# ActiveVisionLab/gaussctrl

Hardware: AMD Instinct MI355X
Metric: edited views/sec @512x512 (ControlNet denoise + splat render+bwd) (higher is better)
Workload: dtype bf16

## Files before the change

### gaussctrl_amd/csrc/dn_gemm.hip

```cpp
#include "dn_gemm_kernels.h"

namespace {

struct GemmVariant {
    int force_mt;
    int use8;
    int convsplit;
    bool no_wg2, no_persist, full_epilogue, no_lean_ln, tap_outer;
    int forced_pw, slice_mt, epi_abl;
    int undefined;
};
GemmVariant decode_variant(int kv)
{
    const auto bit = [kv](int b) { return (kv & b) != 0; };
    const auto field = [kv](int mask, int shift) { return (kv & mask) >> shift; };
    constexpr int flags = GC_GEMM_VAR_K4_ONLY | GC_GEMM_VAR_FORCE_K8 | GC_GEMM_VAR_NO_CONV_SLICES | GC_GEMM_VAR_NO_SMALL_CONV_SLICES | GC_GEMM_VAR_NO_WG2 |
                          GC_GEMM_VAR_NO_PERSIST | GC_GEMM_VAR_FULL_EPILOGUE | GC_GEMM_VAR_NO_LEAN_LN | GC_GEMM_VAR_TAP_OUTER;
    return {field(GC_GEMM_VAR_MT_MASK, GC_GEMM_VAR_MT_SHIFT), bit(GC_GEMM_VAR_K4_ONLY) ? 0 : bit(GC_GEMM_VAR_FORCE_K8) ? 2 : 1,
            bit(GC_GEMM_VAR_NO_CONV_SLICES) ? 0 : bit(GC_GEMM_VAR_NO_SMALL_CONV_SLICES) ? 1 : 2,
            bit(GC_GEMM_VAR_NO_WG2), bit(GC_GEMM_VAR_NO_PERSIST), bit(GC_GEMM_VAR_FULL_EPILOGUE), bit(GC_GEMM_VAR_NO_LEAN_LN), bit(GC_GEMM_VAR_TAP_OUTER),
            field(GC_GEMM_VAR_PW_MASK, GC_GEMM_VAR_PW_SHIFT), field(GC_GEMM_VAR_SLICE_MT_MASK, GC_GEMM_VAR_SLICE_MT_SHIFT), field(GC_GEMM_VAR_EPI_ABL_MASK, GC_GEMM_VAR_EPI_ABL_SHIFT),
            kv & ~(flags | GC_GEMM_VAR_MT_MASK | GC_GEMM_VAR_PW_MASK | GC_GEMM_VAR_SLICE_MT_MASK | GC_GEMM_VAR_EPI_ABL_MASK)};
}

int choose_splits(int64_t blocks, int nk)
{
    if (blocks >= 128 || nk < 32) return 1;
    int s = (int)((448 + blocks - 1) / blocks);
    if (s > nk / 8) s = nk / 8;
    if (s > 16) s = 16;
    return s < 2 ? 1 : s;
}

int choose_mt(int64_t M, int64_t N, int ntw, bool forced)
{
    const int64_t nbn = (N + 32 * ntw - 1) / (32 * ntw);
    if (((M + 127) / 128) * nbn < 96 && !forced) return 0;
    int best = 2;
    int64_t best_cost = -1;
    for (int mt = 2; mt <= 4; ++mt) {
        const int64_t tiles = ((M + 64 * mt - 1) / (64 * mt)) * nbn;
        const int64_t cost = ((tiles + 255) / 256) * (mt + 1);
        if (best_cost < 0 || cost < best_cost || (cost == best_cost && mt == 4)) { best = mt; best_cost = cost; }
    }
    return best;
}

int choose_pw(int64_t nbm, int64_t nbn, int64_t total_wgs, int conc, int64_t bm, int64_t bn, bool conv)
{
    int64_t r = total_wgs / 8 < 1 ? 1 : total_wgs / 8;
    if (r > conc) r = conc;
    const int64_t tiles = nbm * nbn;
    if (r >= tiles) return 0;
    const int64_t ca = conv ? bm : 9 * bm, cw = 9 * bn;
    int best = 0;
    int64_t best_cost = -1;
    for (int64_t pw = nbn; pw >= 1; --pw) {
        const int64_t per = nbm * pw;
        const int64_t cols = std::min<int64_t>(nbn, pw * ((r + per - 1) / per)), rows = std::min<int64_t>(nbm, (r + pw - 1) / pw);
        const int64_t cost = rows * ca + cols * cw;
        if (best_cost < 0 || cost < best_cost) { best = pw == nbn ? 0 : (int)pw; best_cost = cost; }
    }
    return best;
}

int pw_of(const gc_gemm_desc *d, const GemmVariant &v, int64_t nbm, int64_t nbn, int64_t total_wgs, int conc, int64_t bm, int64_t bn)
{
    if (v.forced_pw) return v.forced_pw - 1;
    return choose_pw(nbm, nbn, total_wgs, conc, bm, bn, d->mode == 1);
}

void plan(const gc_gemm_desc *d, int *ntw, int *splits, int *tps)
{
    *ntw = (d->N % 160 == 0 && d->N % 128 != 0 && !d->geglu) ? 5 : 4;
    if (d->softmax_keys > 0) *ntw = 5;
    const int bn = 32 * *ntw;
    const int64_t Msel = d->plan_rows > 0 ? d->plan_rows : d->M;
    const int64_t blocks = ((Msel + BM - 1) / BM) * ((d->N + bn - 1) / bn);
    const int nk = (int)((d->K + BK - 1) / BK);
    *splits = (d->geglu || d->w_set_rows > 0 || d->softmax_keys > 0) ? 1 : choose_splits(blocks, nk);
    *tps = (nk + *splits - 1) / *splits;
    *splits = (nk + *tps - 1) / *tps;
}


struct SelQ { int ntw, mt, splits, tps; };
void select_fp8(const gc_gemm_desc *d, const GemmVariant &v, SelQ *o, bool assume_ws)
{
    const int force_mt = v.force_mt;
    o->ntw = (d->N % 160 == 0 && d->N % 128 != 0 && !d->geglu) ? 5 : 4;
    int mt = force_mt ? force_mt : choose_mt(d->M, d->N, o->ntw, true);
    if (o->ntw == 5) mt = 2; else if (mt > 3) mt = 3;
    if (mt < 2) mt = 2;
    const int nkq = (int)(d->K / 128);
    o->splits = 1; o->tps = nkq;
    const bool plain = !d->geglu && !d->out_t && !d->out_fp8 && !d->out_f32 && d->out && !d->ln_row_stats && !d->out_row_stats && !d->out_group_stats && d->act == 0;
    const int64_t Msel = d->plan_rows > 0 ? d->plan_rows : d->M;
    const int64_t nbn = (d->N + 32 * o->ntw - 1) / (32 * o->ntw), tiles = ((Msel + 127) / 128) * nbn;
    if (plain && !force_mt && v.convsplit && tiles <= 128 && nkq >= 16) {
        int s = (int)std::min<int64_t>(tiles < 96 ? (256 + tiles - 1) / tiles : 256 / tiles, nkq / 8);
        if (s > 16) s = 16;
        if (s >= 2 && (assume_ws || (d->workspace && d->workspace_bytes >= sizeof(float) * (size_t)s * (size_t)d->M * (size_t)d->N))) {
            mt = 2; o->tps = (nkq + s - 1) / s; o->splits = (nkq + o->tps - 1) / o->tps;
        }
    }
    o->mt = mt;
}
}

extern "C" size_t gc_dn_gemm_workspace_bytes(const gc_gemm_desc *d)
{
    if (!d || d->M <= 0 || d->N <= 0 || d->K <= 0) return 0;
    if (d->fp8) {
        if (d->K % 128 != 0) return 0;
        const GemmVariant v = decode_variant(d->kernel_variant);
        SelQ q;
        select_fp8(d, v, &q, true);
        return q.splits > 1 ? sizeof(float) * (size_t)q.splits * (size_t)d->M * (size_t)d->N : 0;
    }
    int ntw, splits, tps;
    plan(d, &ntw, &splits, &tps);
    return splits > 1 ? sizeof(float) * (size_t)splits * (size_t)d->M * (size_t)d->N : 0;
}

namespace {
int ln_lean_kind(const gc_gemm_desc *d, const GemmVariant &v)
{
    if (v.no_lean_ln || d->fp8 || d->mode != 0 || d->K % 64 != 0 || d->out_group_stats || d->out_chan_parts || d->N < 4) return 0;
    if (d->out_row_stats && !d->ln_row_stats)
        return (!d->geglu && d->act == 0 && !d->out_f32 && !d->out_t && d->out && (!d->rowvec || d->rows_per_batch >= 256)) ? 1 : 0;
    if (d->ln_row_stats && !d->out_row_stats) return d->softmax_keys > 0 ? 3 : 2;
    return 0;
}
struct Sel { int mode, ntw, splits, tps, mt8; };
int select(const gc_gemm_desc *d, const GemmVariant &v, Sel *o, bool want_parts)
{
    int mode = 0;
    if (d->mode == 1) mode = (d->Cin % 64 == 0) ? 2 : 1;
    int ntw, splits, tps;
    plan(d, &ntw, &splits, &tps);
    if (splits > 1 && (!d->workspace || d->workspace_bytes < sizeof(float) * (size_t)splits * (size_t)d->M * (size_t)d->N)) {
        splits = 1; tps = (int)((d->K + BK - 1) / BK);
    }
    const int bn = 32 * ntw;
    const int64_t nbn = (d->N + bn - 1) / bn;
    const int nk_host = (int)((d->K + BK - 1) / BK);
    const int force_mt = v.force_mt, use8 = v.use8;
    o->mode = mode; o->ntw = ntw; o->splits = splits; o->tps = tps; o->mt8 = 0;
    if (use8 && d->zeros) {
        const int64_t Msel = d->plan_rows > 0 ? d->plan_rows : d->M;
        int mt = force_mt ? force_mt : choose_mt(Msel, d->N, ntw, use8 == 2);
        if (mt && !force_mt && Msel != d->M) mt = choose_mt(d->M, d->N, ntw, true);
        const int64_t tiles8 = ((Msel + 127) / 128) * nbn;
        const bool small = tiles8 < 96;
        if (!mt && mode == 0 && !force_mt) mt = 2;
        if (mode == 0 && !force_mt && ntw == 4 && d->K % 64 == 0 && !d->geglu && !d->out_t && !v.no_wg2 &&
            (!(d->ln_row_stats || d->out_row_stats || d->out_group_stats) || ln_lean_kind(d, v)) && !want_parts) {
            const int64_t t1 = ((d->M + 63) / 64) * nbn, t2 = ((d->M + 127) / 128) * nbn;
            if (mt == 2 && t2 <= 256 && t1 <= 512 && t1 > 128 && nk_host <= 24) mt = 1;
        }
        if (d->w_set_rows > 0 && mt) {
            int pick = 0;
            const int cand[5] = {mt, 4, 3, 2, (ntw == 4 && d->softmax_keys == 0) ? 1 : 2};
            for (int c = 0; c < 5 && !pick; ++c) if (d->w_set_rows % (64 * cand[c]) == 0) pick = cand[c];
            mt = pick ? pick : mt;
        }
        const bool want_split = !force_mt && use8 != 2 && !d->geglu && d->w_set_rows == 0 && d->softmax_keys == 0 && d->workspace && tiles8 <= 128 && (mode == 0 ? (!small || nk_host >= 24) : (v.convsplit >= (small ? 2 : 1)));
        int s8 = 1, tps8 = nk_host;
        if (want_split) {
            const bool img8 = mode != 0 && !small && d->Ho * d->Wo <= 64 && Msel % 256 == 0;
            const int mts = (v.slice_mt >= 2 && v.slice_mt <= 4) ? v.slice_mt : (img8 ? 4 : ((mode != 0 && !small) ? 3 : 2));
            const int64_t tiles_s = ((Msel + 64 * mts - 1) / (64 * mts)) * nbn;
            s8 = (int)std::min<int64_t>(std::max<int64_t>(256 / tiles_s, 2), nk_host / 12);
            if (s8 >= 2 && d->workspace_bytes >= sizeof(float) * (size_t)s8 * (size_t)d->M * (size_t)d->N) {
                mt = mts; tps8 = (nk_host + s8 - 1) / s8; s8 = (nk_host + tps8 - 1) / tps8;
            } else s8 = 1;
        }
        if (splits > 1 && s8 == 1 && !force_mt && use8 != 2) mt = 0;
        if (mt) { o->mt8 = mt; o->splits = s8; o->tps = tps8; }
    }
    return 0;
}
}

extern "C" int gc_dn_gemm_row_stat_slots(const gc_gemm_desc *d)
{
    if (!d || d->M <= 0 || d->N <= 0 || d->K <= 0) return 0;
    if (d->fp8) { const int ntw = (d->N % 160 == 0 && d->N % 128 != 0) ? 5 : 4; return (int)((d->N + 16 * ntw - 1) / (16 * ntw)); }
    const GemmVariant v = decode_variant(d->kernel_variant);
    Sel sel;
    select(d, v, &sel, false);
    return sel.splits > 1 ? (int)((d->N / 4 + 63) / 64) : (int)((d->N + 16 * sel.ntw - 1) / (16 * sel.ntw));
}

namespace {
void chan_parts_layout(const gc_gemm_desc *d, const GemmVariant &v, const Sel &sel, int64_t *rows, int *nslab, int *col_tile)
{
    *rows = 0; *nslab = 0; *col_tile = 0;
    const int64_t rpb = d->rows_per_batch;
    if (d->fp8) {
        SelQ q;
        select_fp8(d, v, &q, false);
        if (d->K % 128 != 0 || rpb < 256 || rpb % 32 != 0 || d->M % rpb != 0 || d->gn_groups < 1 || d->N % d->gn_groups != 0) return;
        const int64_t cpg = d->N / d->gn_groups;
        if (q.splits > 1) {
            if (cpg > 64) return;
            *rows = CS_RB; *nslab = (int)(rpb / CS_RB); *col_tile = 64;
            return;
        }
        const bool lean = d->mode == 1 && !d->upsample && !d->geglu && !d->out_t && !d->out_fp8 && !d->out_f32 && d->out && d->act == 0 &&
                          !d->ln_row_stats && !d->out_row_stats && !d->out_group_stats;
        const int64_t bm = 64 * q.mt;
        if (!lean || bm > rpb || cpg > 32 * q.ntw) return;
        *rows = bm;
        *nslab = (int)(rpb % bm == 0 ? rpb / bm : (rpb + bm - 1) / bm + 1);
        *col_tile = 32 * q.ntw;
        return;
    }
    if (d->geglu || d->act != 0 || d->out_t || !d->out || d->out_f32 || d->ln_row_stats || d->out_row_stats || d->out_group_stats) return;
    if (rpb < 256 || rpb % 32 != 0 || d->M % rpb != 0) return;
    if (d->gn_groups < 1 || d->N % d->gn_groups != 0) return;
    const int64_t cpg = d->N / d->gn_groups;
    if (sel.splits > 1) {
        if (cpg > 64) return;
        *rows = CS_RB; *nslab = (int)(rpb / CS_RB); *col_tile = 64;
        return;
    }
    if (!sel.mt8) return;
    if ((d->mode == 1 && d->upsample) || (d->mode == 0 && d->K % 64 != 0)) return;
    const int64_t bm = 64 * (sel.mt8 < 2 ? 2 : sel.mt8);
    if (bm > rpb || cpg > 32 * sel.ntw) return;
    *rows = bm;
    *nslab = (int)(rpb % bm == 0 ? rpb / bm : (rpb + bm - 1) / bm + 1);
    *col_tile = 32 * sel.ntw;
}
}

extern "C" int gc_dn_gemm_chan_parts_layout(const gc_gemm_desc *d, int64_t *rows_per_slab, int *nslab, int *col_tile)
{
    GC_REQUIRE(d && rows_per_slab && nslab && col_tile, "null argument");
    *rows_per_slab = 0; *nslab = 0; *col_tile = 0;
    if (d->M <= 0 || d->N <= 0 || d->K <= 0 || d->rows_per_batch <= 0) return GC_OK;
    const GemmVariant v = decode_variant(d->kernel_variant);
    Sel sel;
    select(d, v, &sel, true);
    chan_parts_layout(d, v, sel, rows_per_slab, nslab, col_tile);
    return GC_OK;
}

namespace {
struct Route { Sel sel; int lnk, persist; };
void route(const gc_gemm_desc *d, const GemmVariant &v, Route *r)
{
    Sel &sel = r->sel;
    select(d, v, &sel, d->out_chan_parts != nullptr);
    if (d->out_chan_parts && sel.mt8 == 1) sel.mt8 = 2;
    const bool fuse = d->ln_row_stats || d->out_row_stats || d->out_group_stats;
    r->lnk = (sel.mt8 && sel.splits == 1) ? ln_lean_kind(d, v) : 0;
    r->persist = 0;
    if (sel.mt8 == 4 && sel.ntw == 4 && sel.mode == 0 && sel.splits == 1 && d->K % 64 == 0 && d->K <= 64 * 24 && (!fuse || r->lnk == 2) && !d->out_chan_parts &&
        !d->rowvec && !d->out_t && !d->out_f32 && d->out && d->act != 2 && !v.no_persist) {
        const int64_t tiles = ((d->M + 255) / 256) * ((d->N + 32 * sel.ntw - 1) / (32 * sel.ntw));
        if (tiles > 256) r->persist = 256;
    }
}
}

extern "C" int gc_dn_gemm_selection(const gc_gemm_desc *d, gc_gemm_selection *out)
{
    GC_REQUIRE(d && out, "null argument");
    GC_REQUIRE(d->M > 0 && d->N > 0 && d->K > 0, "empty problem");
    const GemmVariant v = decode_variant(d->kernel_variant);
    if (const int rc = refuse_variant_bits(__func__, v.undefined)) return rc;
    *out = gc_gemm_selection{};
    int64_t rows = 0; int ns = 0, ct = 0;
    if (d->fp8) {
        GC_REQUIRE(d->K % 128 == 0, "fp8: K % 128 == 0");
        SelQ q;
        select_fp8(d, v, &q, false);
        out->kernel = GC_GEMM_SEL_FP8; out->m_tiles = q.mt; out->splits = q.splits; out->ntw = q.ntw;
        if (d->out_chan_parts) {
            chan_parts_layout(d, v, Sel{}, &rows, &ns, &ct);
            out->parts = rows > 0 ? (q.splits > 1 ? 1 : 2) : -1;
        }
        return GC_OK;
    }
    Route r;
    route(d, v, &r);
    out->kernel = !r.sel.mt8 ? GC_GEMM_SEL_K4 : r.sel.splits > 1 ? GC_GEMM_SEL_K8_SLICED : GC_GEMM_SEL_K8;
    out->m_tiles = r.sel.mt8; out->splits = r.sel.splits; out->ntw = r.sel.ntw; out->ln_kind = r.lnk; out->persist = r.persist;
    if (d->out_chan_parts) {
        chan_parts_layout(d, v, r.sel, &rows, &ns, &ct);
        out->parts = rows > 0 ? (r.sel.splits > 1 ? 1 : 2) : -1;
    }
    return GC_OK;
}

extern "C" int gc_dn_gemm(const gc_gemm_desc *d, void *stream)
{
    GC_REQUIRE(d && d->W && d->A, "null descriptor / operand");
    GC_REQUIRE(d->M > 0 && d->N > 0 && d->K > 0, "empty problem");
    GC_REQUIRE(d->K % 8 == 0, "K must be a multiple of 8 (pad channels on the host)");
    GC_REQUIRE(d->N % 4 == 0, "N must be a multiple of 4 (pad output channels on the host)");
    GC_REQUIRE(d->dtype == DT_BF16 || d->dtype == DT_F16, "dtype must be 0 (bf16) or 1 (f16)");
    const GemmVariant v = decode_variant(d->kernel_variant);
    if (const int rc = refuse_variant_bits(__func__, v.undefined)) return rc;
    GemmArgs g;
    g.pw = 0;
    g.M = d->M; g.N = d->N; g.K = d->K; g.A = d->A; g.lda = d->lda;
    g.B = d->B; g.Hi = d->Hi; g.Wi = d->Wi; g.Cin = d->Cin; g.Ho = d->Ho; g.Wo = d->Wo; g.stride = d->stride; g.ups = d->upsample; g.pad = d->pad_lo;
    g.W = d->W; g.bias = d->bias; g.rowvec = d->rowvec; g.ld_rowvec = d->ld_rowvec;
    g.rows_per_batch = d->rows_per_batch > 0 ? d->rows_per_batch : 1;
    g.residual = d->residual; g.ldr = d->ldr; g.out_scale = d->out_scale; g.act = d->act; g.geglu = d->geglu;
    g.out = d->out; g.ldc = d->ldc; g.out_f32 = d->out_f32; g.out_t = d->out_t; g.ldt = d->ldt; g.t_batch_stride = d->t_batch_stride; g.t_col0 = d->t_col0;
    g.row_stats = d->ln_row_stats; g.row_stat_slots = d->ln_row_stat_slots > 0 ? d->ln_row_stat_slots : 1;
    g.colsum = d->ln_colsum; g.ln_eps = d->ln_eps; g.ln_inv_k = 1.f / (float)d->K;
    g.out_row_stats = d->out_row_stats; g.out_group_stats = d->out_group_stats; g.gn_groups = d->gn_groups;
    g.gn_cpg = d->gn_groups > 0 ? (int)(d->N / d->gn_groups) : 1;
    g.w_scale = (const unsigned char *)d->w_scale; g.a_scale = d->a_scale;
    g.out_fp8 = d->out_fp8; g.out_qscale = d->out_fp8 > 0 ? exp2f((float)(127 - d->out_fp8)) : 1.f;
    GC_REQUIRE(d->out_fp8 >= 0 && d->out_fp8 < 255, "out_fp8 must be 0 (off) or an E8M0 byte 1 .. 254");
    GC_REQUIRE(!d->out_fp8 || (d->fp8 && d->mode == 0 && d->out && !d->out_f32 && !d->out_t && !d->out_chan_parts && !d->ln_row_stats && !d->out_row_stats &&
                               !d->out_group_stats && d->ldc % 4 == 0),
               "out_fp8: an fp8 linear with a plain output (no fp32 / transposed output, no statistics, no LayerNorm fold), ldc % 4 == 0");
    g.dbg = v.epi_abl;
    g.conv_korder = v.tap_outer ? 0 : 1;
    g.w_set_rows = d->w_set_rows; g.w_set_stride = d->w_set_stride; g.sm_keys = d->softmax_keys;
    GC_REQUIRE(d->w_set_rows >= 0 && d->softmax_keys >= 0 && d->softmax_keys <= 80, "bad weight-set / softmax arguments");
    GC_REQUIRE(!d->softmax_keys || (d->ln_row_stats && d->N % 80 == 0 && d->out && !d->out_f32 && !d->out_t && !d->geglu && !d->residual && d->act == 0),
               "softmax_keys: a LayerNorm-folded linear with N % 80 == 0 and a plain 2-byte output");
    GC_REQUIRE((d->ln_row_stats == nullptr) == (d->ln_colsum == nullptr), "ln_row_stats and ln_colsum must be given together");
    GC_REQUIRE(!d->ln_row_stats || d->mode == 0, "LayerNorm folding applies to linear GEMMs");
    GC_REQUIRE(!(d->out_row_stats || d->out_group_stats) || (!d->geglu && !d->out_t && d->out), "output statistics need a plain (non-GEGLU, non-transposed) output");
    GC_REQUIRE(!d->out_group_stats || (g.rows_per_batch % 16 == 0 && d->gn_groups >= 1 && d->gn_groups <= GS_MAXG && d->N % d->gn_groups == 0),
               "out_group_stats needs rows_per_batch % 16 == 0 and 1 <= gn_groups <= 32 dividing N");
    if (d->mode == 1) {
        GC_REQUIRE(d->Cin % 8 == 0 && d->K == 9 * (int64_t)d->Cin, "conv3x3: K must be 9*Cin with Cin % 8 == 0");
        GC_REQUIRE(d->M == (int64_t)d->B * d->Ho * d->Wo, "conv3x3: M must be B*Ho*Wo");
        GC_REQUIRE(d->pad_lo == 0 || d->pad_lo == 1, "conv3x3: pad_lo must be 0 or 1");
    } else {
        GC_REQUIRE(d->lda >= d->K && d->lda % 8 == 0, "linear: lda must be >= K and a multiple of 8");
    }
    GC_REQUIRE((d->mode == 1 ? (int64_t)d->B * d->Hi * d->Wi * d->Cin : d->M * d->lda) < ((int64_t)1 << 31) && (int64_t)d->N * d->K < ((int64_t)1 << 31),
               "operand too large for 32-bit element offsets: split the batch");
    if (d->geglu) GC_REQUIRE(d->N % 32 == 0 && !d->out_t, "geglu needs N % 32 == 0");
    GC_REQUIRE(v.force_mt <= 4, "kernel_variant: MT must be 0 .. 4");
    Route rt;
    route(d, v, &rt);
    const Sel &sel = rt.sel;
    g.chan_parts = d->out_chan_parts; g.cp_nslab = 0; g.cp_rows = 0;
    if (d->out_chan_parts) {
        int64_t rows; int ns, ct;
        chan_parts_layout(d, v, sel, &rows, &ns, &ct);
        GC_REQUIRE(rows > 0, "out_chan_parts: this problem cannot produce channel partials (see gc_dn_gemm_chan_parts_layout)");
        g.cp_nslab = ns; g.cp_rows = (int)rows;
    }
    if (fuse_of(g) && sel.mt8) {
        const bool upsampled = d->mode == 1 && d->upsample, ragged = d->mode == 0 && d->K % 64 != 0;
        GC_REQUIRE(!upsampled && !ragged, "row / group statistics and LayerNorm folding: not with upsample-fused convs or K % 64 != 0 linears");
    }
    hipStream_t s = gc::S(stream);
    g.zeros = d->zeros;
    if (d->fp8) {
        GC_REQUIRE(d->zeros && d->w_scale, "fp8: zeros page and per-row weight scales are required");
        GC_REQUIRE(d->K % 128 == 0, "fp8: K % 128 == 0");
        GC_REQUIRE(!(d->geglu || d->out_t) || (d->mode == 0 && !fuse_of(g)), "fp8: GEGLU / transposed output on linears with the plain epilogue only");
        GC_REQUIRE(d->mode == 0 || (d->Cin % 128 == 0 && !d->upsample), "fp8 conv: Cin (padded) % 128 == 0, no fused upsample");
        GC_REQUIRE(d->mode == 1 || d->lda % 16 == 0, "fp8 linear: lda % 16 == 0");
        GC_REQUIRE((int64_t)d->N * d->K < ((int64_t)1 << 31) && (d->mode == 1 ? (int64_t)d->B * d->Hi * d->Wi * d->Cin : d->M * d->lda) < ((int64_t)1 << 31), "fp8: 32-bit offsets");
        SelQ q;
        select_fp8(d, v, &q, false);
        const int ntw = q.ntw, mt = q.mt;
        g.splits = q.splits; g.tiles_per_split = q.tps; g.ws = q.splits > 1 ? (float *)d->workspace : nullptr;
        GC_REQUIRE(!d->out_chan_parts || q.splits > 1 || (d->mode == 1 && !fuse_of(g)), "fp8: channel partials come from k-sliced problems and fast convs");
        const int64_t nbn_q = (d->N + 32 * ntw - 1) / (32 * ntw), nbm_q = (d->M + 64 * mt - 1) / (64 * mt);
        const dim3 gq((unsigned)(nbm_q * nbn_q), (unsigned)q.splits);
        g.pw = pw_of(d, v, nbm_q, nbn_q, nbm_q * nbn_q * q.splits, 32, 64 * mt, 32 * ntw);
        dn_gemm_launch_fp8(g, d->dtype, d->mode == 1 ? 2 : 3, ntw, mt, gq, s);
        if (q.splits > 1) { if (g.chan_parts) dn_gemm_launch_splitk_epilogue_cs(g, d->dtype, s); else dn_gemm_launch_splitk_epilogue(g, d->dtype, s); }
        return gc::check_launch("gc_dn_gemm(fp8)");
    }
    g.splits = sel.splits; g.tiles_per_split = sel.tps; g.ws = (float *)d->workspace;
    const int bn = 32 * sel.ntw;
    const int64_t nbn = (d->N + bn - 1) / bn;
    g.persist = rt.persist;
    const int lnk = rt.lnk;
    if (d->w_set_rows > 0 || d->softmax_keys > 0) {
        GC_REQUIRE(lnk != 0, "weight sets / softmax_keys need a lean LayerNorm-fold problem (K % 64 == 0 linear with ln_row_stats or out_row_stats, no forced variant)");
        GC_REQUIRE(d->w_set_rows == 0 || (d->w_set_rows % (64 * sel.mt8) == 0 && d->M % d->w_set_rows == 0), "w_set_rows must be a multiple of the row tile and divide M");
    }
    if (sel.mt8) {
        const int64_t nbm8 = (d->M + 64 * sel.mt8 - 1) / (64 * sel.mt8);
        const dim3 grid8((unsigned)(nbm8 * nbn), (unsigned)sel.splits);
        g.pw = pw_of(d, v, nbm8, nbn, g.persist ? 8 * 32 : nbm8 * nbn * sel.splits, sel.mt8 == 1 ? 64 : 32, 64 * sel.mt8, bn);
        if (lnk) dn_gemm_launch_ln(g, d->dtype, lnk, lean_of(g, sel.mode) && g.persist == 0, sel.ntw, sel.mt8, grid8, s);
        else if (fuse_of(g)) dn_gemm_launch_fuse(g, d->dtype, sel.mode, sel.ntw, sel.mt8 < 2 ? 2 : sel.mt8, grid8, s);
        else if (g.chan_parts && sel.splits == 1) dn_gemm_launch_cs(g, d->dtype, sel.mode, sel.ntw, sel.mt8, grid8, s);
        else if (lean_of(g, sel.mode) && g.persist == 0 && !v.full_epilogue) dn_gemm_launch_lean(g, d->dtype, sel.mode, sel.ntw, sel.mt8, grid8, s);
        else dn_gemm_launch_plain(g, d->dtype, sel.mode, sel.ntw, sel.mt8, grid8, s);
    } else {
        const int64_t nbm = (d->M + BM - 1) / BM;
        const dim3 grid((unsigned)(nbm * nbn), (unsigned)sel.splits);
        g.pw = pw_of(d, v, nbm, nbn, nbm * nbn * sel.splits, 64, BM, bn);
        if (fuse_of(g)) dn_gemm_launch_fuse(g, d->dtype, sel.mode, sel.ntw, 0, grid, s); else dn_gemm_launch_plain(g, d->dtype, sel.mode, sel.ntw, 0, grid, s);
    }
    if (sel.splits > 1) { if (g.chan_parts) dn_gemm_launch_splitk_epilogue_cs(g, d->dtype, s); else dn_gemm_launch_splitk_epilogue(g, d->dtype, s); }
    return gc::check_launch("gc_dn_gemm");
}
```

### gaussctrl_amd/csrc/dn_gemm_kernels.h

```cpp
#pragma once
#include "dn_common.h"
#include <type_traits>

namespace dng {
struct GemmArgs {
    int64_t M, N, K;
    const void *A; int64_t lda;
    int B, Hi, Wi, Cin, Ho, Wo, stride, ups, pad;
    const void *W;
    const float *bias;
    const float *rowvec; int64_t ld_rowvec; int64_t rows_per_batch;
    const void *residual; int64_t ldr;
    float out_scale;
    int act, geglu;
    void *out; int64_t ldc; int out_f32;
    void *out_t; int64_t ldt; int64_t t_batch_stride; int64_t t_col0;
    int splits; int tiles_per_split;
    int persist;
    float *ws;
    const void *zeros;
    const float *row_stats; int row_stat_slots; const float *colsum; float ln_eps, ln_inv_k;
    float *out_row_stats;
    float *out_group_stats;
    int gn_groups, gn_cpg;
    const unsigned char *w_scale;
    int a_scale;
    int out_fp8; float out_qscale;
    int dbg;
    float *chan_parts; int cp_nslab; int cp_rows;
    int64_t w_set_rows, w_set_stride;
    int pw;
    int sm_keys;
    int conv_korder;
};

__device__ __forceinline__ void tile_coords(int64_t bid, int nbm, int nbn, int pw, int64_t &mblk, int64_t &nblk)
{
    if (pw <= 0 || pw >= nbn) { mblk = bid / nbn; nblk = bid % nbn; return; }
    const int64_t per = (int64_t)nbm * pw, p = bid / per, within = bid - p * per;
    const int64_t w = (nbn - p * pw) < pw ? (nbn - p * pw) : pw;
    mblk = within / w; nblk = p * pw + within % w;
}
__device__ __forceinline__ void wg_tile(const GemmArgs &g, int nbm, int nbn, int64_t &mblk, int64_t &nblk, int &slice)
{
    const int64_t tiles = gridDim.x, total = tiles * gridDim.y, lin = blockIdx.x + tiles * blockIdx.y;
    const int64_t xcd = lin & 7, qq = total >> 3, rr = total & 7;
    const int64_t L = (xcd < rr ? xcd * (qq + 1) : rr * (qq + 1) + (xcd - rr) * qq) + (lin >> 3);
    slice = (int)(L / tiles);
    tile_coords(L - (int64_t)slice * tiles, nbm, nbn, g.pw, mblk, nblk);
}
}

namespace {
using namespace dn;
using dng::GemmArgs;

template <int I, int N, class F> __device__ __forceinline__ void static_for(F &&f)
{
    if constexpr (I < N) {
        f(std::integral_constant<int, I>{});
        static_for<I + 1, N>(f);
    }
}

constexpr int BM = 128, BK = 64;
constexpr int NT = 256;


constexpr int GS_SLOTS = 20, GS_MAXG = 32;

__device__ __forceinline__ float row16_sum(float v)
{
    v += __builtin_bit_cast(float, __builtin_amdgcn_update_dpp(0, __builtin_bit_cast(int, v), 0x128, 0xf, 0xf, false));
    v += __builtin_bit_cast(float, __builtin_amdgcn_update_dpp(0, __builtin_bit_cast(int, v), 0x124, 0xf, 0xf, false));
    v += __builtin_bit_cast(float, __builtin_amdgcn_update_dpp(0, __builtin_bit_cast(int, v), 0x122, 0xf, 0xf, false));
    v += __builtin_bit_cast(float, __builtin_amdgcn_update_dpp(0, __builtin_bit_cast(int, v), 0x121, 0xf, 0xf, false));
    return v;
}

__device__ __forceinline__ int lds_off(int r, int c) { return r * 128 + ((c ^ ((r >> 1) & 7)) << 4); }

template <class T>
__device__ __forceinline__ void epilogue_store(const GemmArgs &g, int64_t m, int64_t n, int64_t on, float *v, const float *gate, const uint2 *res_pre = nullptr)
{
    const int64_t bidx = g.rowvec ? m / g.rows_per_batch : 0;
    if (g.row_stats) {
        float2 rs = make_float2(0.f, 0.f);
        for (int sl = 0; sl < g.row_stat_slots; ++sl) {
            const float2 t = *reinterpret_cast<const float2 *>(g.row_stats + ((int64_t)sl * g.M + m) * 2);
            rs.x += t.x; rs.y += t.y;
        }
        const float mean = rs.x * g.ln_inv_k, rstd = rsqrtf(fmaxf(rs.y * g.ln_inv_k - mean * mean, 0.f) + g.ln_eps);
#pragma unroll
        for (int r = 0; r < 4; ++r) v[r] = rstd * (v[r] - mean * g.colsum[n + r]);
    }
#pragma unroll
    for (int r = 0; r < 4; ++r) {
        if (g.bias) v[r] += g.bias[n + r];
        if (g.rowvec) v[r] += g.rowvec[bidx * g.ld_rowvec + n + r];
    }
    if (g.geglu) {
#pragma unroll
        for (int r = 0; r < 4; ++r) {
            float gt = gate[r];
            if (g.bias) gt += g.bias[n + 16 + r];
            v[r] = v[r] * gelu_erf(gt);
        }
    }
    if (g.act == 1) {
#pragma unroll
        for (int r = 0; r < 4; ++r) v[r] = silu(v[r]);
    } else if (g.act == 2) {
#pragma unroll
        for (int r = 0; r < 4; ++r) v[r] = fminf(fmaxf(v[r] * 0.5f + 0.5f, 0.f), 1.f);
    }
#pragma unroll
    for (int r = 0; r < 4; ++r) v[r] *= g.out_scale;
    if (g.residual) {
        const uint2 rr = res_pre ? *res_pre : *reinterpret_cast<const uint2 *>((const unsigned char *)g.residual + (m * g.ldr + on) * 2);
        v[0] += T::to_f((unsigned short)(rr.x & 0xffff)); v[1] += T::to_f((unsigned short)(rr.x >> 16));
        v[2] += T::to_f((unsigned short)(rr.y & 0xffff)); v[3] += T::to_f((unsigned short)(rr.y >> 16));
    }
    const bool to_t = g.out_t && on >= g.t_col0;
    const uint2 pk = make_uint2(pack2<T>(v[0], v[1]), pack2<T>(v[2], v[3]));
    if (g.out && !(to_t && g.t_col0 > 0)) {
        if (g.out_f32)
            *reinterpret_cast<float4 *>((float *)g.out + m * g.ldc + on) = make_float4(v[0], v[1], v[2], v[3]);
        else
            *reinterpret_cast<uint2 *>((unsigned char *)g.out + (m * g.ldc + on) * 2) = pk;
    }
    if (to_t) {
        const int64_t b = m / g.rows_per_batch, tok = m - b * g.rows_per_batch;
        unsigned short *o = (unsigned short *)g.out_t + b * g.t_batch_stride + tok;
#pragma unroll
        for (int r = 0; r < 4; ++r) o[(on - g.t_col0 + r) * g.ldt] = T::from_f(v[r]);
    }
    if (!g.out_f32) {
        v[0] = T::to_f((unsigned short)(pk.x & 0xffff)); v[1] = T::to_f((unsigned short)(pk.x >> 16));
        v[2] = T::to_f((unsigned short)(pk.y & 0xffff)); v[3] = T::to_f((unsigned short)(pk.y >> 16));
    }
}

template <int BM>
__device__ __forceinline__ void row_stats_prologue(const GemmArgs &g, int64_t m_base, float *srow)
{
    const int t = threadIdx.x, r = t & 255, half = t >> 8;
    if (t < 2 * BM) srow[t] = 0.f;
    asm volatile("s_waitcnt lgkmcnt(0)" ::: "memory");
    __builtin_amdgcn_s_barrier();
    if (r < BM) {
        const int64_t m = m_base + r < g.M ? m_base + r : g.M - 1;
        const float *rp = g.row_stats + m * 2;
        const int64_t st = g.M * 2;
        float sx = 0.f, sy = 0.f;
        int sl = half;
        for (; sl + 6 < g.row_stat_slots; sl += 8) {
            const float2 a = *reinterpret_cast<const float2 *>(rp + sl * st), b = *reinterpret_cast<const float2 *>(rp + (sl + 2) * st);
            const float2 c = *reinterpret_cast<const float2 *>(rp + (sl + 4) * st), d = *reinterpret_cast<const float2 *>(rp + (sl + 6) * st);
            sx += (a.x + b.x) + (c.x + d.x); sy += (a.y + b.y) + (c.y + d.y);
        }
        for (; sl < g.row_stat_slots; sl += 2) {
            const float2 a = *reinterpret_cast<const float2 *>(rp + sl * st);
            sx += a.x; sy += a.y;
        }
        __hip_atomic_fetch_add(srow + 2 * r, sx, __ATOMIC_RELAXED, __HIP_MEMORY_SCOPE_WORKGROUP);
        __hip_atomic_fetch_add(srow + 2 * r + 1, sy, __ATOMIC_RELAXED, __HIP_MEMORY_SCOPE_WORKGROUP);
    }
    asm volatile("s_waitcnt vmcnt(0) lgkmcnt(0)" ::: "memory");
}

template <class T, int NTW, int MT, int NTHREADS>
__device__ __forceinline__ void wave_epilogue(const GemmArgs &g, f32x4 (&acc)[NTW][MT], int64_t m_base, int64_t m_wave, int64_t n_wave, int lane,
                                              unsigned char *smem, const float *srow = nullptr, int slice = 0)
{
    const int fr = lane & 15, fc = lane >> 4;
    const int64_t n_lane = n_wave + fc * 4;
    if (g.splits > 1) {
#pragma unroll
        for (int mt = 0; mt < MT; ++mt) {
            const int64_t m = m_wave + mt * 16 + fr;
            if (m >= g.M) continue;
#pragma unroll
            for (int nt = 0; nt < NTW; ++nt) {
                const int64_t n = n_lane + nt * 16;
                if (n < g.N)
                    *reinterpret_cast<float4 *>(g.ws + ((int64_t)slice * g.M + m) * g.N + n) =
                        make_float4(acc[nt][mt][0], acc[nt][mt][1], acc[nt][mt][2], acc[nt][mt][3]);
            }
        }
        return;
    }
    if (g.out_group_stats) {
        asm volatile("s_waitcnt lgkmcnt(0)" ::: "memory");
        __builtin_amdgcn_s_barrier();
        for (int idx = threadIdx.x; idx < GS_SLOTS * GS_MAXG * 2; idx += NTHREADS) reinterpret_cast<float *>(smem)[idx] = 0.f;
        asm volatile("s_waitcnt lgkmcnt(0)" ::: "memory");
        __builtin_amdgcn_s_barrier();
    }
    float4 bia[NTW], csm[NTW];
#pragma unroll
    for (int nt = 0; nt < NTW; ++nt) {
        const int64_t n = n_lane + nt * 16;
        bia[nt] = (g.bias && n < g.N) ? *reinterpret_cast<const float4 *>(g.bias + n) : make_float4(0.f, 0.f, 0.f, 0.f);
        csm[nt] = (g.row_stats && n < g.N) ? *reinterpret_cast<const float4 *>(g.colsum + n) : make_float4(0.f, 0.f, 0.f, 0.f);
    }
    uint2 rs_all[MT][NTW];
#pragma unroll
    for (int mt = 0; mt < MT; ++mt) {
        const int64_t m = m_wave + mt * 16 + fr;
        const bool okm = m < g.M;
        const int64_t mc = okm ? m : 0;
#pragma unroll
        for (int nt = 0; nt < NTW; ++nt) {
            const int64_t n = n_lane + nt * 16;
            const bool okn = okm && n < g.N && !(g.geglu && (nt & 1));
            const int64_t on = g.geglu ? (n_wave + nt * 16) / 2 + fc * 4 : n;
            rs_all[mt][nt] = (g.residual && okn) ? *reinterpret_cast<const uint2 *>((const unsigned char *)g.residual + (mc * g.ldr + on) * 2) : make_uint2(0u, 0u);
        }
    }
    const bool want_cs = g.out_group_stats != nullptr;
    float *red = reinterpret_cast<float *>(smem);
    const int64_t b0 = want_cs ? m_base / g.rows_per_batch : 0;
    float cs[NTW][4], css[NTW][4];
#pragma unroll
    for (int nt = 0; nt < NTW; ++nt)
#pragma unroll
        for (int r = 0; r < 4; ++r) { cs[nt][r] = 0.f; css[nt][r] = 0.f; }
    int64_t cs_b = -1;
    auto flush_cs = [&]() __attribute__((always_inline)) {
        float *rb = red + (cs_b - b0) * (GS_MAXG * 2);
#pragma unroll
        for (int nt = 0; nt < NTW; ++nt) {
            const int64_t n = n_lane + nt * 16;
#pragma unroll
            for (int r = 0; r < 4; ++r) {
                const float a = (g.dbg & 4) ? cs[nt][r] : row16_sum(cs[nt][r]), b = (g.dbg & 4) ? css[nt][r] : row16_sum(css[nt][r]);
                if (fr == 0 && n + r < g.N && !(g.dbg & 2)) {
                    const int gi = (int)(n + r) / g.gn_cpg;
                    __hip_atomic_fetch_add(rb + 2 * gi, a, __ATOMIC_RELAXED, __HIP_MEMORY_SCOPE_WORKGROUP);
                    __hip_atomic_fetch_add(rb + 2 * gi + 1, b, __ATOMIC_RELAXED, __HIP_MEMORY_SCOPE_WORKGROUP);
                }
                cs[nt][r] = 0.f; css[nt][r] = 0.f;
            }
        }
    };
#pragma unroll
    for (int mt = 0; mt < MT; ++mt) {
        const int64_t m = m_wave + mt * 16 + fr;
        const int64_t m_tile = m_wave + mt * 16;
        if (m_tile >= g.M) break;
        const bool okm = m < g.M;
        if (want_cs) {
            const int64_t b = m_tile / g.rows_per_batch;
            if (cs_b >= 0 && b != cs_b) flush_cs();
            cs_b = b;
        }
        const uint2 *rs = rs_all[mt];
        float mean = 0.f, rstd = 1.f;
        if (g.row_stats) {
            float sx = 0.f, sy = 0.f;
            if (srow) {
                const float2 t = *reinterpret_cast<const float2 *>(srow + 2 * (okm ? (int)(m - m_base) : 0));
                sx = t.x; sy = t.y;
            } else {
                const float *rp = g.row_stats + (okm ? m : 0) * 2;
                for (int sl = 0; sl < g.row_stat_slots; ++sl) {
                    const float2 t = *reinterpret_cast<const float2 *>(rp + (int64_t)sl * g.M * 2);
                    sx += t.x; sy += t.y;
                }
            }
            mean = sx * g.ln_inv_k;
            rstd = rsqrtf(fmaxf(sy * g.ln_inv_k - mean * mean, 0.f) + g.ln_eps);
        }
        float4 rv[NTW];
        const int64_t bidx = (g.rowvec && okm) ? m / g.rows_per_batch : 0;
#pragma unroll
        for (int nt = 0; nt < NTW; ++nt) {
            const int64_t n = n_lane + nt * 16;
            rv[nt] = (g.rowvec && n < g.N) ? *reinterpret_cast<const float4 *>(g.rowvec + bidx * g.ld_rowvec + n) : make_float4(0.f, 0.f, 0.f, 0.f);
        }
        float rsum = 0.f, rsq = 0.f;
#pragma unroll
        for (int nt = 0; nt < NTW; ++nt) {
            const int64_t n = n_lane + nt * 16;
            if (n >= g.N) continue;
            if (g.geglu && (nt & 1)) continue;
            float a0 = acc[nt][mt][0], a1 = acc[nt][mt][1], a2 = acc[nt][mt][2], a3 = acc[nt][mt][3];
            if (g.row_stats) {
                a0 = rstd * (a0 - mean * csm[nt].x); a1 = rstd * (a1 - mean * csm[nt].y);
                a2 = rstd * (a2 - mean * csm[nt].z); a3 = rstd * (a3 - mean * csm[nt].w);
            }
            float v[4] = {a0 + bia[nt].x + rv[nt].x, a1 + bia[nt].y + rv[nt].y, a2 + bia[nt].z + rv[nt].z, a3 + bia[nt].w + rv[nt].w};
            int64_t on = n;
            if (g.geglu) {
                constexpr int NP = NTW - 1;
                const int np = nt + 1 < NTW ? nt + 1 : NP;
                float g0 = acc[np][mt][0], g1 = acc[np][mt][1], g2 = acc[np][mt][2], g3 = acc[np][mt][3];
                if (g.row_stats) {
                    g0 = rstd * (g0 - mean * csm[np].x); g1 = rstd * (g1 - mean * csm[np].y);
                    g2 = rstd * (g2 - mean * csm[np].z); g3 = rstd * (g3 - mean * csm[np].w);
                }
                v[0] *= gelu_erf(g0 + bia[np].x); v[1] *= gelu_erf(g1 + bia[np].y);
                v[2] *= gelu_erf(g2 + bia[np].z); v[3] *= gelu_erf(g3 + bia[np].w);
                on = (n_wave + nt * 16) / 2 + fc * 4;
            }
            if (g.act == 1) {
#pragma unroll
                for (int r = 0; r < 4; ++r) v[r] = silu(v[r]);
            } else if (g.act == 2) {
#pragma unroll
                for (int r = 0; r < 4; ++r) v[r] = fminf(fmaxf(v[r] * 0.5f + 0.5f, 0.f), 1.f);
            }
#pragma unroll
            for (int r = 0; r < 4; ++r) v[r] *= g.out_scale;
            if (g.residual) {
                v[0] += T::to_f((unsigned short)(rs[nt].x & 0xffff)); v[1] += T::to_f((unsigned short)(rs[nt].x >> 16));
                v[2] += T::to_f((unsigned short)(rs[nt].y & 0xffff)); v[3] += T::to_f((unsigned short)(rs[nt].y >> 16));
            }
            if (!okm) continue;
            const bool to_t = g.out_t && on >= g.t_col0;
            const uint2 pk = make_uint2(pack2<T>(v[0], v[1]), pack2<T>(v[2], v[3]));
            if (g.out && !(to_t && g.t_col0 > 0)) {
                if (g.out_f32)
                    *reinterpret_cast<float4 *>((float *)g.out + m * g.ldc + on) = make_float4(v[0], v[1], v[2], v[3]);
                else
                    *reinterpret_cast<uint2 *>((unsigned char *)g.out + (m * g.ldc + on) * 2) = pk;
            }
            if (to_t) {
                const int64_t b = m / g.rows_per_batch, tok = m - b * g.rows_per_batch;
                unsigned short *o = (unsigned short *)g.out_t + b * g.t_batch_stride + tok;
#pragma unroll
                for (int r = 0; r < 4; ++r) o[(on - g.t_col0 + r) * g.ldt] = T::from_f(v[r]);
            }
            if (g.out_row_stats || want_cs) {
                float t[4];
                if (g.out_f32) { t[0] = v[0]; t[1] = v[1]; t[2] = v[2]; t[3] = v[3]; }
                else {
                    t[0] = T::to_f((unsigned short)(pk.x & 0xffff)); t[1] = T::to_f((unsigned short)(pk.x >> 16));
                    t[2] = T::to_f((unsigned short)(pk.y & 0xffff)); t[3] = T::to_f((unsigned short)(pk.y >> 16));
                }
#pragma unroll
                for (int r = 0; r < 4; ++r) {
                    rsum += t[r]; rsq += t[r] * t[r];
                    cs[nt][r] += t[r]; css[nt][r] += t[r] * t[r];
                }
            }
        }
        if (g.out_row_stats && n_wave < g.N) {
            rsum += __shfl_xor(rsum, 16, 64); rsq += __shfl_xor(rsq, 16, 64);
            rsum += __shfl_xor(rsum, 32, 64); rsq += __shfl_xor(rsq, 32, 64);
            const int64_t slot = n_wave / (16 * NTW);
            if (fc == 0 && okm) *reinterpret_cast<float2 *>(g.out_row_stats + (slot * g.M + m) * 2) = make_float2(rsum, rsq);
        }
    }
    if (want_cs) {
        if (cs_b >= 0) flush_cs();
        asm volatile("s_waitcnt lgkmcnt(0)" ::: "memory");
        __builtin_amdgcn_s_barrier();
        for (int idx = threadIdx.x; idx < GS_SLOTS * GS_MAXG * 2; idx += NTHREADS) {
            const float v = red[idx];
            if (v != 0.f && !(g.dbg & 1)) {
                const int sl = idx / (GS_MAXG * 2), rem = idx - sl * (GS_MAXG * 2);
                unsafeAtomicAdd(g.out_group_stats + ((b0 + sl) * g.gn_groups) * 2 + rem, v);
            }
        }
    }
}

template <class T, int MODE, int NTW, bool FUSE>
__global__ __launch_bounds__(NT, 2) void k_gemm(const GemmArgs g)
{
    constexpr int BN = 32 * NTW;
    constexpr int WCH = BN * 8 / NT;
    constexpr int STAGE = BM * 128 + BN * 128;
    extern __shared__ __attribute__((aligned(16))) unsigned char smem[];
    const int tid = threadIdx.x, lane = tid & 63, wid = tid >> 6;
    const int wm = wid >> 1, wn = wid & 1;
    const int nbn = (int)((g.N + BN - 1) / BN);
    int64_t mblk, nblk;
    int slice;
    wg_tile(g, (int)((g.M + BM - 1) / BM), nbn, mblk, nblk, slice);
    const int64_t m_base = mblk * BM, n_base = nblk * BN;
    const int nk = (int)((g.K + BK - 1) / BK);
    const int kt0 = slice * g.tiles_per_split, kt1 = min(nk, kt0 + g.tiles_per_split);
    if (kt0 >= kt1) return;

    int a_row[4], a_chunk[4];
    int a_off[4];
    int a_y[4], a_x[4];
    bool a_ok[4];
    int w_off[WCH];
    bool w_ok[WCH];
#pragma unroll
    for (int i = 0; i < 4; ++i) {
        const int q = tid + NT * i;
        a_row[i] = q >> 3; a_chunk[i] = q & 7;
        const int64_t m = m_base + a_row[i];
        a_ok[i] = m < g.M;
        const int mm = a_ok[i] ? (int)m : 0;
        if (MODE != 0) {
            const int hw = g.Ho * g.Wo;
            const int b = mm / hw;
            const int rem = mm - b * hw;
            const int oy = rem / g.Wo;
            a_y[i] = oy * g.stride - g.pad; a_x[i] = (rem - oy * g.Wo) * g.stride - g.pad;
            a_off[i] = b * g.Hi * g.Wi * g.Cin + (MODE == 2 ? a_chunk[i] * 8 : 0);
            if (MODE == 2 && !g.ups) a_off[i] += (a_y[i] * g.Wi + a_x[i]) * g.Cin;
        } else {
            a_off[i] = mm * (int)g.lda + a_chunk[i] * 8;
            a_y[i] = a_x[i] = 0;
        }
    }
#pragma unroll
    for (int i = 0; i < WCH; ++i) {
        const int q = tid + NT * i;
        const int64_t n = n_base + (q >> 3);
        w_ok[i] = n < g.N;
        w_off[i] = (w_ok[i] ? (int)n : 0) * (int)g.K + (q & 7) * 8;
    }
    const int Hin = g.ups ? g.Hi * 2 : g.Hi, Win = g.ups ? g.Wi * 2 : g.Wi;
    const unsigned char *Ab = (const unsigned char *)g.A, *Wb = (const unsigned char *)g.W;
    const int ktl = kt1 - 1;
    int ld_tap = 0, ld_ci = 0;
    if (MODE == 2) { ld_tap = (kt0 * BK) / g.Cin; ld_ci = kt0 * BK - ld_tap * g.Cin; }

    auto load_tile = [&](int kt, uint4 *ra, uint4 *rw, unsigned &mask) __attribute__((always_inline)) {
        const int kb = kt * BK;
        int dy_u = 0, dx_u = 0, tap_off = 0;
        if (MODE == 2) {
            dy_u = ld_tap / 3; dx_u = ld_tap - dy_u * 3;
            tap_off = g.ups ? ld_ci : (dy_u * g.Wi + dx_u) * g.Cin + ld_ci;
            if (kt < ktl) { ld_ci += BK; if (ld_ci >= g.Cin) { ld_ci -= g.Cin; ++ld_tap; } }
        }
        unsigned mk = 0;
#pragma unroll
        for (int i = 0; i < 4; ++i) {
            bool ok;
            int off;
            if (MODE == 2) {
                int yi = a_y[i] + dy_u, xi = a_x[i] + dx_u;
                ok = a_ok[i] && (unsigned)yi < (unsigned)Hin && (unsigned)xi < (unsigned)Win;
                off = a_off[i] + tap_off;
                if (g.ups) off += ((yi >> 1) * g.Wi + (xi >> 1)) * g.Cin;
            } else if (MODE == 1) {
                const int k0 = kb + a_chunk[i] * 8;
                const int kc = k0 < (int)g.K ? k0 : 0;
                const int tap = kc / g.Cin;
                const int ci = kc - tap * g.Cin;
                const int dy = tap / 3, dx = tap - dy * 3;
                int yi = a_y[i] + dy, xi = a_x[i] + dx;
                ok = a_ok[i] && k0 < (int)g.K && (unsigned)yi < (unsigned)Hin && (unsigned)xi < (unsigned)Win;
                if (g.ups) { yi >>= 1; xi >>= 1; }
                off = a_off[i] + (yi * g.Wi + xi) * g.Cin + ci;
            } else {
                ok = a_ok[i] && (kb + a_chunk[i] * 8) < (int)g.K;
                off = a_off[i] + kb;
            }
            ra[i] = *reinterpret_cast<const uint4 *>(Ab + (size_t)(unsigned)((ok ? off : 0) * 2));
            mk |= (ok ? 1u : 0u) << i;
        }
#pragma unroll
        for (int i = 0; i < WCH; ++i) {
            const int q = tid + NT * i;
            const bool ok = w_ok[i] && (kb + (q & 7) * 8) < (int)g.K;
            rw[i] = *reinterpret_cast<const uint4 *>(Wb + (size_t)(unsigned)((ok ? w_off[i] + kb : 0) * 2));
            mk |= (ok ? 1u : 0u) << (8 + i);
        }
        mask = mk;
    };
    constexpr unsigned FULL = 0xFu | (((1u << WCH) - 1u) << 8);
    int sa_off[4], sw_off[WCH];
#pragma unroll
    for (int i = 0; i < 4; ++i) sa_off[i] = lds_off(a_row[i], a_chunk[i]);
#pragma unroll
    for (int i = 0; i < WCH; ++i) { const int q = tid + NT * i; sw_off[i] = BM * 128 + lds_off(q >> 3, q & 7); }
    auto store_tile = [&](int buf, uint4 *ra, uint4 *rw, unsigned mask) __attribute__((always_inline)) {
        unsigned char *sa = smem + buf * STAGE;
        if (!__all(mask == FULL)) {
#pragma unroll
            for (int i = 0; i < 4; ++i) {
                const unsigned km = 0u - ((mask >> i) & 1u);
                ra[i] = make_uint4(ra[i].x & km, ra[i].y & km, ra[i].z & km, ra[i].w & km);
            }
#pragma unroll
            for (int i = 0; i < WCH; ++i) {
                const unsigned km = 0u - ((mask >> (8 + i)) & 1u);
                rw[i] = make_uint4(rw[i].x & km, rw[i].y & km, rw[i].z & km, rw[i].w & km);
            }
        }
#pragma unroll
        for (int i = 0; i < 4; ++i) *reinterpret_cast<uint4 *>(sa + sa_off[i]) = ra[i];
#pragma unroll
        for (int i = 0; i < WCH; ++i) *reinterpret_cast<uint4 *>(sa + sw_off[i]) = rw[i];
    };

    f32x4 acc[NTW][4];
#pragma unroll
    for (int a = 0; a < NTW; ++a)
#pragma unroll
        for (int b = 0; b < 4; ++b) acc[a][b] = f32x4{0.f, 0.f, 0.f, 0.f};
    const int fr = lane & 15, fc = lane >> 4;
    const int swz = (fr >> 1) & 7;
    const int fx0 = ((fc ^ swz) << 4), fx1 = (((fc + 4) ^ swz) << 4);
    const int aw0 = BM * 128 + (wn * (16 * NTW) + fr) * 128, aa0 = (wm * 64 + fr) * 128;
    auto compute = [&](int buf) __attribute__((always_inline)) {
        const unsigned char *sb = smem + buf * STAGE;
#pragma unroll
        for (int ks = 0; ks < 2; ++ks) {
            const int fx = ks ? fx1 : fx0;
            uint4 fw[NTW], fa[4];
#pragma unroll
            for (int t = 0; t < NTW; ++t) fw[t] = *reinterpret_cast<const uint4 *>(sb + aw0 + fx + t * 2048);
#pragma unroll
            for (int t = 0; t < 4; ++t) fa[t] = *reinterpret_cast<const uint4 *>(sb + aa0 + fx + t * 2048);
#pragma unroll
            for (int nt = 0; nt < NTW; ++nt)
#pragma unroll
                for (int mt = 0; mt < 4; ++mt) acc[nt][mt] = T::mfma(fw[nt], fa[mt], acc[nt][mt]);
        }
    };

    uint4 raA[4], rwA[WCH], raB[4], rwB[WCH];
    unsigned mkA = 0, mkB = 0;
    load_tile(kt0, raA, rwA, mkA);
    load_tile(min(kt0 + 1, ktl), raB, rwB, mkB);
    store_tile(0, raA, rwA, mkA);
    __syncthreads();
    for (int kt = kt0; kt < kt1; kt += 2) {
        load_tile(min(kt + 2, ktl), raA, rwA, mkA);
        compute(0);
        store_tile(1, raB, rwB, mkB);
        __syncthreads();
        if (kt + 1 >= kt1) break;
        load_tile(min(kt + 3, ktl), raB, rwB, mkB);
        compute(1);
        store_tile(0, raA, rwA, mkA);
        __syncthreads();
    }

    if constexpr (FUSE) {
        wave_epilogue<T, NTW, 4, NT>(g, acc, m_base, m_base + wm * 64, n_base + wn * (16 * NTW), lane, smem, nullptr, slice);
        return;
    }
    const int64_t n_lane = n_base + wn * (16 * NTW) + fc * 4;
    if (g.splits > 1) {
#pragma unroll
        for (int mt = 0; mt < 4; ++mt) {
            const int64_t m = m_base + wm * 64 + mt * 16 + fr;
            if (m >= g.M) continue;
#pragma unroll
            for (int nt = 0; nt < NTW; ++nt) {
                const int64_t n = n_lane + nt * 16;
                if (n < g.N)
                    *reinterpret_cast<float4 *>(g.ws + ((int64_t)slice * g.M + m) * g.N + n) =
                        make_float4(acc[nt][mt][0], acc[nt][mt][1], acc[nt][mt][2], acc[nt][mt][3]);
            }
        }
        return;
    }
    float4 bia[NTW];
#pragma unroll
    for (int nt = 0; nt < NTW; ++nt) {
        const int64_t n = n_lane + nt * 16;
        bia[nt] = (g.bias && n < g.N) ? *reinterpret_cast<const float4 *>(g.bias + n) : make_float4(0.f, 0.f, 0.f, 0.f);
    }
    uint2 rs_all[4][NTW];
#pragma unroll
    for (int mt = 0; mt < 4; ++mt) {
        const int64_t m = m_base + wm * 64 + mt * 16 + fr;
        const bool okm = m < g.M;
        const int64_t mc = okm ? m : 0;
#pragma unroll
        for (int nt = 0; nt < NTW; ++nt) {
            const int64_t n = n_lane + nt * 16;
            const bool okn = okm && n < g.N && !(g.geglu && (nt & 1));
            const int64_t on = g.geglu ? (n_base + wn * (16 * NTW) + nt * 16) / 2 + fc * 4 : n;
            rs_all[mt][nt] = (g.residual && okn) ? *reinterpret_cast<const uint2 *>((const unsigned char *)g.residual + (mc * g.ldr + on) * 2) : make_uint2(0u, 0u);
        }
    }
#pragma unroll
    for (int mt = 0; mt < 4; ++mt) {
        const int64_t m = m_base + wm * 64 + mt * 16 + fr;
        if (m >= g.M) continue;
        const uint2 *rs = rs_all[mt];
        float4 rv[NTW];
        const int64_t bidx = g.rowvec ? m / g.rows_per_batch : 0;
#pragma unroll
        for (int nt = 0; nt < NTW; ++nt) {
            const int64_t n = n_lane + nt * 16;
            rv[nt] = (g.rowvec && n < g.N) ? *reinterpret_cast<const float4 *>(g.rowvec + bidx * g.ld_rowvec + n) : make_float4(0.f, 0.f, 0.f, 0.f);
        }
#pragma unroll
        for (int nt = 0; nt < NTW; ++nt) {
            const int64_t n = n_lane + nt * 16;
            if (n >= g.N) continue;
            if (g.geglu && (nt & 1)) continue;
            float v[4] = {acc[nt][mt][0] + bia[nt].x + rv[nt].x, acc[nt][mt][1] + bia[nt].y + rv[nt].y,
                          acc[nt][mt][2] + bia[nt].z + rv[nt].z, acc[nt][mt][3] + bia[nt].w + rv[nt].w};
            int64_t on = n;
            if (g.geglu) {
                constexpr int NP = NTW - 1;
                const int np = nt + 1 < NTW ? nt + 1 : NP;
                v[0] *= gelu_erf(acc[np][mt][0] + bia[np].x); v[1] *= gelu_erf(acc[np][mt][1] + bia[np].y);
                v[2] *= gelu_erf(acc[np][mt][2] + bia[np].z); v[3] *= gelu_erf(acc[np][mt][3] + bia[np].w);
                on = (n_base + wn * (16 * NTW) + nt * 16) / 2 + fc * 4;
            }
            if (g.act == 1) {
#pragma unroll
                for (int r = 0; r < 4; ++r) v[r] = silu(v[r]);
            } else if (g.act == 2) {
#pragma unroll
                for (int r = 0; r < 4; ++r) v[r] = fminf(fmaxf(v[r] * 0.5f + 0.5f, 0.f), 1.f);
            }
#pragma unroll
            for (int r = 0; r < 4; ++r) v[r] *= g.out_scale;
            if (g.residual) {
                v[0] += T::to_f((unsigned short)(rs[nt].x & 0xffff)); v[1] += T::to_f((unsigned short)(rs[nt].x >> 16));
                v[2] += T::to_f((unsigned short)(rs[nt].y & 0xffff)); v[3] += T::to_f((unsigned short)(rs[nt].y >> 16));
            }
            const bool to_t = g.out_t && on >= g.t_col0;
            if (g.out && !(to_t && g.t_col0 > 0)) {
                if (g.out_f32)
                    *reinterpret_cast<float4 *>((float *)g.out + m * g.ldc + on) = make_float4(v[0], v[1], v[2], v[3]);
                else
                    *reinterpret_cast<uint2 *>((unsigned char *)g.out + (m * g.ldc + on) * 2) = make_uint2(pack2<T>(v[0], v[1]), pack2<T>(v[2], v[3]));
            }
            if (to_t) {
                const int64_t b = m / g.rows_per_batch, tok = m - b * g.rows_per_batch;
                unsigned short *o = (unsigned short *)g.out_t + b * g.t_batch_stride + tok;
#pragma unroll
                for (int r = 0; r < 4; ++r) o[(on - g.t_col0 + r) * g.ldt] = T::from_f(v[r]);
            }
        }
    }
}

__device__ __forceinline__ void glds16(const void *gsrc, unsigned lds_dst)
{
    unsigned keep;
    asm volatile("s_mov_b32 %0, m0\n\ts_mov_b32 m0, %2\n\ts_nop 0\n\tglobal_load_lds_dwordx4 %1, off\n\ts_mov_b32 m0, %0"
                 : "=&s"(keep) : "v"(gsrc), "s"(lds_dst) : "memory");
}

__device__ __forceinline__ void glds16_s(const void *sbase, unsigned voff, unsigned lds_dst)
{
    asm volatile("s_mov_b32 m0, %2\n\ts_nop 0\n\tglobal_load_lds_dwordx4 %0, %1" :: "v"(voff), "s"(sbase), "s"(lds_dst) : "memory");
}

template <class T, int MODE, int NTW, int MT, bool FUSE, bool CS = false, bool LEAN_ = false, int LNV = 0>
__global__ __launch_bounds__(512, MT <= 2 ? 2 : 1) void k_gemm8(const GemmArgs g)
{
    static_assert(!(FUSE && CS), "one statistics epilogue at a time");
    static_assert(LNV == 0 || (!FUSE && !CS && MODE == 3), "lean LayerNorm fold: K % 64 == 0 linears on the non-FUSE epilogues");
    static_assert(LNV != 1 || LEAN_, "row partials come from the lean epilogue");
    static_assert(LNV != 3 || (NTW == 5 && !LEAN_), "softmax-heads epilogue: one 80-column head block per wave column");
    constexpr bool LNIN = LNV >= 2;
    constexpr bool LEAN = LEAN_ || CS;
    constexpr int BM = 64 * MT;
    constexpr bool CONVF = MODE == 2 || MODE == 4, UPS = MODE == 4;
    constexpr int BN = 32 * NTW;
    constexpr int STAGE = BM * 128 + BN * 128;
    constexpr int NS = 3;
    constexpr int AG = BM / 8, WG = BN / 8;
    constexpr int AI = AG / 8, WI = (WG + 7) / 8;
    extern __shared__ __attribute__((aligned(16))) unsigned char smem[];
    const int tid = threadIdx.x, lane = tid & 63;
    const int wid = __builtin_amdgcn_readfirstlane(tid >> 6);
    const int wm = wid >> 1, wn = wid & 1;
    const int nbn = (int)((g.N + BN - 1) / BN);
    int64_t mblk, nblk;
    int slice;
    wg_tile(g, (int)((g.M + BM - 1) / BM), nbn, mblk, nblk, slice);
    const int64_t m_base = mblk * BM, n_base = nblk * BN;
    const int nk_all = (int)((g.K + BK - 1) / BK);
    const int kt0 = slice * g.tiles_per_split;
    const int nk = min(nk_all, kt0 + g.tiles_per_split) - kt0;
    const unsigned lds0 = (unsigned)(size_t)(__attribute__((address_space(3))) unsigned char *)smem;
    float *srow = reinterpret_cast<float *>(smem + NS * STAGE);
    if constexpr (FUSE) {
        if (g.row_stats && g.splits == 1) row_stats_prologue<BM>(g, m_base, srow);
    }
    float *ctab = reinterpret_cast<float *>(smem + NS * STAGE);
    if constexpr (CS) {
        for (int i = tid; i < 4 * BN; i += 512) ctab[i] = 0.f;
    }

    const int lr = lane >> 3, ls = lane & 7;
    int a_off[AI], a_y[AI], a_x[AI], a_ck[AI];
    bool a_ok[AI];
#pragma unroll
    for (int i = 0; i < AI; ++i) {
        const int row = (wid + 8 * i) * 8 + lr;
        a_ck[i] = ls ^ ((row >> 1) & 7);
        const int64_t m = m_base + row;
        a_ok[i] = m < g.M;
        const int mm = a_ok[i] ? (int)m : 0;
        if (MODE == 1 || CONVF) {
            const int hw = g.Ho * g.Wo;
            const int b = mm / hw;
            const int rem = mm - b * hw;
            const int oy = rem / g.Wo;
            a_y[i] = oy * g.stride - g.pad; a_x[i] = (rem - oy * g.Wo) * g.stride - g.pad;
            a_off[i] = b * g.Hi * g.Wi * g.Cin + (CONVF ? a_ck[i] * 8 : 0);
            if (MODE == 2) a_off[i] += (a_y[i] * g.Wi + a_x[i]) * g.Cin;
        } else {
            a_off[i] = mm * (int)g.lda + a_ck[i] * 8;
            if (MODE == 3) a_off[i] = (int)(m < g.M ? m : g.M - 1) * (int)g.lda + a_ck[i] * 8;
            a_y[i] = a_x[i] = 0;
        }
    }
    int w_off[WI], w_ck[WI];
    bool w_ok[WI];
#pragma unroll
    for (int i = 0; i < WI; ++i) {
        const int grp = wid + 8 * i;
        const int row = grp * 8 + lr;
        w_ck[i] = ls ^ ((row >> 1) & 7);
        const int64_t n = n_base + row;
        w_ok[i] = grp < WG && n < g.N;
        w_off[i] = (w_ok[i] ? (int)n : 0) * (int)g.K + w_ck[i] * 8;
        if (MODE == 3) w_off[i] = (int)(n < g.N ? n : g.N - 1) * (int)g.K + w_ck[i] * 8;
    }
    const bool ups = CONVF ? UPS : (g.ups != 0);
    const int Hin = ups ? g.Hi * 2 : g.Hi, Win = ups ? g.Wi * 2 : g.Wi;
    const unsigned char *a_ptr[AI];
    unsigned a_vm[AI];
    if (MODE == 2) {
#pragma unroll
        for (int i = 0; i < AI; ++i) {
            a_ptr[i] = (const unsigned char *)g.A + (int64_t)a_off[i] * 2;
            unsigned vm = 0;
#pragma unroll
            for (int tp = 0; tp < 9; ++tp) {
                const int yi = a_y[i] + tp / 3, xi = a_x[i] + tp % 3;
                if (a_ok[i] && (unsigned)yi < (unsigned)Hin && (unsigned)xi < (unsigned)Win) vm |= 1u << tp;
            }
            a_vm[i] = vm;
        }
    }
    const int64_t wset = (LNV != 0 && g.w_set_rows > 0) ? m_base / g.w_set_rows : 0;
    const unsigned char *Ab = (const unsigned char *)g.A, *Wb = (const unsigned char *)g.W + (LNV != 0 ? wset * g.w_set_stride * 2 : 0);
    const unsigned char *Zp = (const unsigned char *)g.zeros;
    const bool tap_inner = CONVF && g.conv_korder != 0;
    int ld_tap = 0, ld_ci = 0;
    if (CONVF && kt0 > 0) {
        if (tap_inner) { ld_tap = kt0 % 9; ld_ci = (kt0 / 9) * BK; }
        else { ld_tap = (kt0 * BK) / g.Cin; ld_ci = kt0 * BK - ld_tap * g.Cin; }
    }

    struct TileSrc { int kb, dy_u, dx_u, tap_off, tap; unsigned sbase; };
    auto issue_begin = [&](int kt, int stage) __attribute__((always_inline)) -> TileSrc {
        TileSrc t;
        t.kb = (kt0 + kt) * BK; t.dy_u = 0; t.dx_u = 0; t.tap_off = 0; t.tap = 0;
        if (CONVF) {
            t.tap = ld_tap;
            t.kb = __builtin_amdgcn_readfirstlane(ld_tap * g.Cin + ld_ci);
            t.dy_u = ld_tap / 3; t.dx_u = ld_tap - t.dy_u * 3;
            t.tap_off = UPS ? ld_ci : (t.dy_u * g.Wi + t.dx_u) * g.Cin + ld_ci;
            if (tap_inner) { if (++ld_tap == 9) { ld_tap = 0; ld_ci += BK; } }
            else { ld_ci += BK; if (ld_ci >= g.Cin) { ld_ci -= g.Cin; ++ld_tap; } }
        }
        t.sbase = lds0 + stage * STAGE;
        return t;
    };
    auto issue_a = [&](const TileSrc &t, int i) __attribute__((always_inline)) {
        const unsigned dst = t.sbase + (unsigned)((wid + 8 * i) * 1024);
        if (MODE == 3) { glds16_s(Ab + (size_t)t.kb * 2, (unsigned)(a_off[i] * 2), dst); return; }
        if (MODE == 2) {
            const bool okm = (a_vm[i] >> t.tap) & 1u;
            glds16(okm ? a_ptr[i] + (int64_t)t.tap_off * 2 : Zp, dst);
            return;
        }
        bool ok;
        int off;
        if (MODE == 4) {
            int yi = a_y[i] + t.dy_u, xi = a_x[i] + t.dx_u;
            ok = a_ok[i] && (unsigned)yi < (unsigned)Hin && (unsigned)xi < (unsigned)Win;
            off = a_off[i] + t.tap_off;
            off += ((yi >> 1) * g.Wi + (xi >> 1)) * g.Cin;
        } else if (MODE == 1) {
            const int k0 = t.kb + a_ck[i] * 8;
            const int kc = k0 < (int)g.K ? k0 : 0;
            const int tap = kc / g.Cin;
            const int ci = kc - tap * g.Cin;
            const int dy = tap / 3, dx = tap - dy * 3;
            int yi = a_y[i] + dy, xi = a_x[i] + dx;
            ok = a_ok[i] && k0 < (int)g.K && (unsigned)yi < (unsigned)Hin && (unsigned)xi < (unsigned)Win;
            if (g.ups) { yi >>= 1; xi >>= 1; }
            off = a_off[i] + (yi * g.Wi + xi) * g.Cin + ci;
        } else {
            ok = a_ok[i] && (t.kb + a_ck[i] * 8) < (int)g.K;
            off = a_off[i] + t.kb;
        }
        const unsigned char *src = ok ? Ab + (size_t)(unsigned)(off * 2) : Zp;
        glds16(src, dst);
    };
    auto issue_w = [&](const TileSrc &t, int i, bool has) __attribute__((always_inline)) {
        if (has) {
            const unsigned dst = t.sbase + (unsigned)(BM * 128 + (wid + 8 * i) * 1024);
            if (MODE == 3 || CONVF) { glds16_s(Wb + (size_t)t.kb * 2, (unsigned)(w_off[i] * 2), dst); return; }
            const bool ok = w_ok[i] && (t.kb + w_ck[i] * 8) < (int)g.K;
            const unsigned char *src = ok ? Wb + (size_t)(unsigned)((w_off[i] + t.kb) * 2) : Zp;
            glds16(src, dst);
        }
    };
    auto issue = [&](int kt, int stage) __attribute__((always_inline)) {
        const TileSrc t = issue_begin(kt, stage);
#pragma unroll
        for (int i = 0; i < AI; ++i) issue_a(t, i);
#pragma unroll
        for (int i = 0; i < WI; ++i) issue_w(t, i, wid + 8 * i < WG);
    };

    f32x4 acc[NTW][MT];
#pragma unroll
    for (int a = 0; a < NTW; ++a)
#pragma unroll
        for (int b = 0; b < MT; ++b) acc[a][b] = f32x4{0.f, 0.f, 0.f, 0.f};
    const int fr = lane & 15, fc = lane >> 4;
    const int swz = (fr >> 1) & 7;
    const int fx0 = ((fc ^ swz) << 4), fx1 = (((fc + 4) ^ swz) << 4);
    const int aw0 = BM * 128 + (wn * (16 * NTW) + fr) * 128, aa0 = (wm * (16 * MT) + fr) * 128;
    struct Frag { uint4 w[NTW], a[MT]; };
    auto load_frag = [&](Frag &f, int stage, int ks) __attribute__((always_inline)) {
        const unsigned char *sb = smem + stage * STAGE;
        const int fx = ks ? fx1 : fx0;
#pragma unroll
        for (int t = 0; t < NTW; ++t) f.w[t] = *reinterpret_cast<const uint4 *>(sb + aw0 + fx + t * 2048);
#pragma unroll
        for (int t = 0; t < MT; ++t) f.a[t] = *reinterpret_cast<const uint4 *>(sb + aa0 + fx + t * 2048);
    };
    constexpr int NMM = NTW * MT, NPC = AI + WI;
    auto block = [&](const Frag &f, Frag &fn, int st_next, int ks_next, bool load_next, const TileSrc &t, auto dma_tag, auto w3_tag) __attribute__((always_inline)) {
        constexpr bool DMA = decltype(dma_tag)::value, W3 = decltype(w3_tag)::value;
        static_for<0, NMM>([&](auto m_) __attribute__((always_inline)) {
            constexpr int m = decltype(m_)::value, nt = m / MT, mt = m % MT;
            acc[nt][mt] = T::mfma(f.w[nt], f.a[mt], acc[nt][mt]);
            if constexpr (m == 0) {
                __builtin_amdgcn_sched_barrier(0);
                if (load_next) load_frag(fn, st_next, ks_next);
                __builtin_amdgcn_sched_barrier(0);
            } else if constexpr (DMA && m >= 2) {
                static_for<0, NPC>([&](auto p_) __attribute__((always_inline)) {
                    constexpr int pp = decltype(p_)::value;
                    if constexpr (m == 2 + (pp * (NMM - 3)) / NPC) {
                        __builtin_amdgcn_sched_barrier(0);
                        if constexpr (pp < AI) issue_a(t, pp); else issue_w(t, pp - AI, (pp - AI) < WI - 1 || W3 || WG % 8 == 0);
                        __builtin_amdgcn_sched_barrier(0);
                    }
                });
            }
        });
    };

    const bool w3 = (wid + 8 * (WI - 1)) < WG;
    Frag f0, f1;
    const TileSrc tnone = {0, 0, 0, 0, 0, 0u};
    auto run = [&](auto w3_tag) __attribute__((always_inline)) {
        constexpr bool W3 = decltype(w3_tag)::value;
        constexpr int GRPW = AI + ((W3 || WG % 8 == 0) ? WI : WI - 1);
        static_assert(2 * GRPW < 64, "vmcnt range");
        auto wait_tiles = [&](auto n_) __attribute__((always_inline)) {
            asm volatile("s_waitcnt vmcnt(%0)" ::"n"(decltype(n_)::value * GRPW) : "memory");
        };
        issue(0, 0);
        if (nk > 1) issue(1, 1);
        if (nk > 2) issue(2, 2);
        if constexpr (LNIN) row_stats_prologue<BM>(g, m_base, srow);
        if (nk > 2) wait_tiles(std::integral_constant<int, 2>{}); else if (nk > 1) wait_tiles(std::integral_constant<int, 1>{}); else wait_tiles(std::integral_constant<int, 0>{});
        __builtin_amdgcn_s_barrier();
        load_frag(f0, 0, 0);
        int st = 0, kt = 0;
        for (; kt + 3 < nk; ++kt) {
            const int st1 = st + 1 == NS ? 0 : st + 1;
            block(f0, f1, st, 1, true, tnone, std::false_type{}, w3_tag);
            wait_tiles(std::integral_constant<int, 1>{});
            asm volatile("s_waitcnt lgkmcnt(0)" ::: "memory");
            __builtin_amdgcn_s_barrier();
            const TileSrc t = issue_begin(kt + 3, st);
            block(f1, f0, st1, 0, true, t, std::true_type{}, w3_tag);
            st = st1;
        }
        for (; kt < nk; ++kt) {
            const int st1 = st + 1 == NS ? 0 : st + 1;
            block(f0, f1, st, 1, true, tnone, std::false_type{}, w3_tag);
            if (kt + 1 < nk) {
                if (kt + 2 < nk) wait_tiles(std::integral_constant<int, 1>{}); else wait_tiles(std::integral_constant<int, 0>{});
                asm volatile("s_waitcnt lgkmcnt(0)" ::: "memory");
                __builtin_amdgcn_s_barrier();
                block(f1, f0, st1, 0, true, tnone, std::false_type{}, w3_tag);
            } else {
                block(f1, f0, st1, 0, false, tnone, std::false_type{}, w3_tag);
            }
            st = st1;
        }
    };
    if (w3) run(std::true_type{}); else run(std::false_type{});

    if constexpr (FUSE) {
        wave_epilogue<T, NTW, MT, 512>(g, acc, m_base, m_base + wm * (16 * MT), n_base + wn * (16 * NTW), lane, smem,
                                       (g.row_stats && g.splits == 1) ? srow : nullptr, slice);
        return;
    }
    const int64_t n_lane = n_base + wn * (16 * NTW) + fc * 4;
    if (g.splits > 1) {
#pragma unroll
        for (int mt = 0; mt < MT; ++mt) {
            const int64_t m = m_base + wm * (16 * MT) + mt * 16 + fr;
            if (m >= g.M) continue;
#pragma unroll
            for (int nt = 0; nt < NTW; ++nt) {
                const int64_t n = n_lane + nt * 16;
                if (n < g.N)
                    *reinterpret_cast<float4 *>(g.ws + ((int64_t)slice * g.M + m) * g.N + n) =
                        make_float4(acc[nt][mt][0], acc[nt][mt][1], acc[nt][mt][2], acc[nt][mt][3]);
            }
        }
        return;
    }
    if constexpr (LNV == 3) {
        const float *biasp = g.bias + wset * g.N, *csp = g.colsum + wset * g.N;
        float4 bia[NTW], csm[NTW];
#pragma unroll
        for (int nt = 0; nt < NTW; ++nt) {
            const int64_t n = n_lane + nt * 16, nc = n < g.N ? n : g.N - 4;
            bia[nt] = *reinterpret_cast<const float4 *>(biasp + nc);
            csm[nt] = *reinterpret_cast<const float4 *>(csp + nc);
        }
#pragma unroll
        for (int mt = 0; mt < MT; ++mt) {
            const int64_t m = m_base + wm * (16 * MT) + mt * 16 + fr;
            const float2 st = *reinterpret_cast<const float2 *>(srow + 2 * (wm * (16 * MT) + mt * 16 + fr));
            const float mean = st.x * g.ln_inv_k, rstd = rsqrtf(fmaxf(st.y * g.ln_inv_k - mean * mean, 0.f) + g.ln_eps);
            float v[NTW][4];
            float mx = -3.0e38f;
#pragma unroll
            for (int nt = 0; nt < NTW; ++nt) {
                v[nt][0] = rstd * (acc[nt][mt][0] - mean * csm[nt].x) + bia[nt].x; v[nt][1] = rstd * (acc[nt][mt][1] - mean * csm[nt].y) + bia[nt].y;
                v[nt][2] = rstd * (acc[nt][mt][2] - mean * csm[nt].z) + bia[nt].z; v[nt][3] = rstd * (acc[nt][mt][3] - mean * csm[nt].w) + bia[nt].w;
#pragma unroll
                for (int r = 0; r < 4; ++r) {
                    const bool key = nt * 16 + fc * 4 + r < g.sm_keys;
                    v[nt][r] = key ? v[nt][r] : -3.0e38f;
                    mx = fmaxf(mx, v[nt][r]);
                }
            }
            mx = fmaxf(mx, __shfl_xor(mx, 16, 64)); mx = fmaxf(mx, __shfl_xor(mx, 32, 64));
            float sum = 0.f;
#pragma unroll
            for (int nt = 0; nt < NTW; ++nt)
#pragma unroll
                for (int r = 0; r < 4; ++r) { v[nt][r] = exp2f(v[nt][r] - mx); sum += v[nt][r]; }
            sum += __shfl_xor(sum, 16, 64); sum += __shfl_xor(sum, 32, 64);
            const float inv = 1.f / sum;
#pragma unroll
            for (int nt = 0; nt < NTW; ++nt) {
                const int64_t n = n_lane + nt * 16;
                if (m < g.M && n < g.N)
                    *reinterpret_cast<uint2 *>((unsigned char *)g.out + (m * g.ldc + n) * 2) =
                        make_uint2(pack2<T>(v[nt][0] * inv, v[nt][1] * inv), pack2<T>(v[nt][2] * inv, v[nt][3] * inv));
            }
        }
        return;
    }
    if constexpr (LEAN) {
        const unsigned char *zp = (const unsigned char *)g.zeros;
        const bool has_b = g.bias != nullptr, has_rv = g.rowvec != nullptr, has_res = g.residual != nullptr;
        const float *biasp = has_b ? g.bias + (LNV != 0 ? wset * g.N : 0) : reinterpret_cast<const float *>(zp);
        const float *rvp = has_rv ? g.rowvec : reinterpret_cast<const float *>(zp);
        const unsigned char *resp = has_res ? (const unsigned char *)g.residual : zp;
        const int64_t bA = m_base / g.rows_per_batch, b_last = (g.M - 1) / g.rows_per_batch;
        const int64_t bB = bA + 1 < b_last ? bA + 1 : b_last;
        const int64_t m_rv = (bA + 1) * g.rows_per_batch;
        float4 bia[NTW], rvA[NTW], rvB[NTW];
        uint2 rs[MT][NTW];
#pragma unroll
        for (int nt = 0; nt < NTW; ++nt) {
            const int64_t n = n_lane + nt * 16, nc = n < g.N ? n : g.N - 4;
            bia[nt] = *reinterpret_cast<const float4 *>(biasp + (has_b ? nc : 0));
            rvA[nt] = *reinterpret_cast<const float4 *>(rvp + (has_rv ? bA * g.ld_rowvec + nc : 0));
            rvB[nt] = *reinterpret_cast<const float4 *>(rvp + (has_rv ? bB * g.ld_rowvec + nc : 0));
        }
#pragma unroll
        for (int mt = 0; mt < MT; ++mt) {
            const int64_t m = m_base + wm * (16 * MT) + mt * 16 + fr, mc = m < g.M ? m : g.M - 1;
#pragma unroll
            for (int nt = 0; nt < NTW; ++nt) {
                const int64_t n = n_lane + nt * 16, nc = n < g.N ? n : g.N - 4;
                rs[mt][nt] = *reinterpret_cast<const uint2 *>(resp + (has_res ? (mc * g.ldr + nc) * 2 : 0));
            }
        }
        float4 csm[LNV == 2 ? NTW : 1];
        if constexpr (LNV == 2) {
#pragma unroll
            for (int nt = 0; nt < NTW; ++nt) {
                const int64_t n = n_lane + nt * 16, nc = n < g.N ? n : g.N - 4;
                csm[nt] = *reinterpret_cast<const float4 *>(g.colsum + wset * g.N + nc);
            }
        }
        uint2 pks[CS ? MT : 1][CS ? NTW : 1];
#pragma unroll
        for (int mt = 0; mt < MT; ++mt) {
            const int64_t m = m_base + wm * (16 * MT) + mt * 16 + fr;
            const bool second = m >= m_rv;
            float mean = 0.f, rstd = 1.f;
            if constexpr (LNV == 2) {
                const float2 st = *reinterpret_cast<const float2 *>(srow + 2 * (wm * (16 * MT) + mt * 16 + fr));
                mean = st.x * g.ln_inv_k;
                rstd = rsqrtf(fmaxf(st.y * g.ln_inv_k - mean * mean, 0.f) + g.ln_eps);
            }
            float rsum = 0.f, rsq = 0.f;
#pragma unroll
            for (int nt = 0; nt < NTW; ++nt) {
                const int64_t n = n_lane + nt * 16;
                const float4 rv = second ? rvB[nt] : rvA[nt];
                float a0 = acc[nt][mt][0], a1 = acc[nt][mt][1], a2 = acc[nt][mt][2], a3 = acc[nt][mt][3];
                if constexpr (LNV == 2) {
                    a0 = rstd * (a0 - mean * csm[nt].x); a1 = rstd * (a1 - mean * csm[nt].y);
                    a2 = rstd * (a2 - mean * csm[nt].z); a3 = rstd * (a3 - mean * csm[nt].w);
                }
                float v[4] = {a0 + bia[nt].x + rv.x, a1 + bia[nt].y + rv.y, a2 + bia[nt].z + rv.z, a3 + bia[nt].w + rv.w};
#pragma unroll
                for (int r = 0; r < 4; ++r) v[r] *= g.out_scale;
                v[0] += T::to_f((unsigned short)(rs[mt][nt].x & 0xffff)); v[1] += T::to_f((unsigned short)(rs[mt][nt].x >> 16));
                v[2] += T::to_f((unsigned short)(rs[mt][nt].y & 0xffff)); v[3] += T::to_f((unsigned short)(rs[mt][nt].y >> 16));
                const uint2 pk = make_uint2(pack2<T>(v[0], v[1]), pack2<T>(v[2], v[3]));
                const bool ok = m < g.M && n < g.N;
                if (ok) *reinterpret_cast<uint2 *>((unsigned char *)g.out + (m * g.ldc + n) * 2) = pk;
                if constexpr (CS) pks[mt][nt] = ok ? pk : make_uint2(0u, 0u);
                if constexpr (LNV == 1) {
                    const float w_ = n < g.N ? 1.f : 0.f;
                    const float t0 = w_ * T::to_f((unsigned short)(pk.x & 0xffff)), t1 = w_ * T::to_f((unsigned short)(pk.x >> 16));
                    const float t2 = w_ * T::to_f((unsigned short)(pk.y & 0xffff)), t3 = w_ * T::to_f((unsigned short)(pk.y >> 16));
                    rsum += (t0 + t1) + (t2 + t3); rsq += (t0 * t0 + t1 * t1) + (t2 * t2 + t3 * t3);
                }
            }
            if constexpr (LNV == 1) {
                rsum += __shfl_xor(rsum, 16, 64); rsq += __shfl_xor(rsq, 16, 64);
                rsum += __shfl_xor(rsum, 32, 64); rsq += __shfl_xor(rsq, 32, 64);
                const int64_t slot = (n_base + wn * (16 * NTW)) / (16 * NTW);
                if (fc == 0 && m < g.M && n_base + wn * (16 * NTW) < g.N)
                    *reinterpret_cast<float2 *>(g.out_row_stats + (slot * g.M + m) * 2) = make_float2(rsum, rsq);
            }
        }
        if constexpr (CS) {
            const int64_t m_split = (m_base / g.rows_per_batch + 1) * g.rows_per_batch;
            const int64_t m_end = m_base + BM < g.M ? m_base + BM : g.M;
            const int npass = m_split < m_end ? 2 : 1;
    #pragma unroll 1
            for (int pass = 0; pass < npass; ++pass) {
                float cs[NTW][4], cq[NTW][4];
    #pragma unroll
                for (int nt = 0; nt < NTW; ++nt)
    #pragma unroll
                    for (int r = 0; r < 4; ++r) { cs[nt][r] = 0.f; cq[nt][r] = 0.f; }
    #pragma unroll
                for (int mt = 0; mt < MT; ++mt) {
                    const int64_t m_tile = m_base + wm * (16 * MT) + mt * 16;
                    const float wgt = ((m_tile >= m_split ? 1 : 0) == pass) ? 1.f : 0.f;
    #pragma unroll
                    for (int nt = 0; nt < NTW; ++nt) {
                        const uint2 pk = pks[mt][nt];
                        const float t0 = wgt != 0.f ? T::to_f((unsigned short)(pk.x & 0xffff)) : 0.f, t1 = wgt != 0.f ? T::to_f((unsigned short)(pk.x >> 16)) : 0.f;
                        const float t2 = wgt != 0.f ? T::to_f((unsigned short)(pk.y & 0xffff)) : 0.f, t3 = wgt != 0.f ? T::to_f((unsigned short)(pk.y >> 16)) : 0.f;
                        cs[nt][0] += t0; cq[nt][0] += t0 * t0; cs[nt][1] += t1; cq[nt][1] += t1 * t1;
                        cs[nt][2] += t2; cq[nt][2] += t2 * t2; cs[nt][3] += t3; cq[nt][3] += t3 * t3;
                    }
                }
                float *tb = ctab + (pass * BN + wn * (16 * NTW) + fc * 4) * 2;
    #pragma unroll
                for (int nt = 0; nt < NTW; ++nt)
    #pragma unroll
                    for (int r = 0; r < 4; ++r) {
                        const float sa = row16_sum(cs[nt][r]), sb = row16_sum(cq[nt][r]);
                        if (fr == 0) {
                            __hip_atomic_fetch_add(tb + (nt * 16 + r) * 2, sa, __ATOMIC_RELAXED, __HIP_MEMORY_SCOPE_WORKGROUP);
                            __hip_atomic_fetch_add(tb + (nt * 16 + r) * 2 + 1, sb, __ATOMIC_RELAXED, __HIP_MEMORY_SCOPE_WORKGROUP);
                        }
                    }
            }
            asm volatile("s_waitcnt lgkmcnt(0)" ::: "memory");
            __builtin_amdgcn_s_barrier();
            const int64_t b0 = m_base / g.rows_per_batch;
            const int cpg = g.gn_cpg, G = (int)(g.N / cpg);
            const int n_hi = (int)(n_base + BN < g.N ? n_base + BN : g.N);
            const int g_first = (int)n_base / cpg, ng = (n_hi - 1) / cpg - g_first + 1;
            for (int i = tid; i < 2 * ng; i += 512) {
                const int slot = i >= ng ? 1 : 0, gg = g_first + i - slot * ng;
                if (slot == 1 && !(m_split < m_end)) continue;
                const int c_lo = gg * cpg > (int)n_base ? gg * cpg : (int)n_base, c_hi = (gg + 1) * cpg < n_hi ? (gg + 1) * cpg : n_hi;
                float s1 = 0.f, s2 = 0.f;
                for (int c = c_lo; c < c_hi; ++c) { const float2 t = *reinterpret_cast<const float2 *>(ctab + (slot * BN + c - (int)n_base) * 2); s1 += t.x; s2 += t.y; }
                const int64_t b = b0 + slot;
                const int64_t slab = mblk - (b * g.rows_per_batch) / BM;
                const int half = gg * cpg < (int)n_base ? 1 : 0;
                *reinterpret_cast<float2 *>(g.chan_parts + ((((b * g.cp_nslab + slab) * G + gg) * 2 + half) * 2)) = make_float2(s1, s2);
            }
        }
    } else {
    float4 bia[NTW], csm[LNV == 2 ? NTW : 1];
#pragma unroll
    for (int nt = 0; nt < NTW; ++nt) {
        const int64_t n = n_lane + nt * 16;
        bia[nt] = (g.bias && n < g.N) ? *reinterpret_cast<const float4 *>(g.bias + n) : make_float4(0.f, 0.f, 0.f, 0.f);
        if constexpr (LNV == 2) csm[nt] = n < g.N ? *reinterpret_cast<const float4 *>(g.colsum + n) : make_float4(0.f, 0.f, 0.f, 0.f);
    }
#pragma unroll
    for (int mt = 0; mt < MT; ++mt) {
        const int64_t m = m_base + wm * (16 * MT) + mt * 16 + fr;
        if (m >= g.M) continue;
        if constexpr (LNV == 2) {
            const float2 st = *reinterpret_cast<const float2 *>(srow + 2 * (wm * (16 * MT) + mt * 16 + fr));
            const float mean = st.x * g.ln_inv_k, rstd = rsqrtf(fmaxf(st.y * g.ln_inv_k - mean * mean, 0.f) + g.ln_eps);
#pragma unroll
            for (int nt = 0; nt < NTW; ++nt) {
                acc[nt][mt][0] = rstd * (acc[nt][mt][0] - mean * csm[nt].x); acc[nt][mt][1] = rstd * (acc[nt][mt][1] - mean * csm[nt].y);
                acc[nt][mt][2] = rstd * (acc[nt][mt][2] - mean * csm[nt].z); acc[nt][mt][3] = rstd * (acc[nt][mt][3] - mean * csm[nt].w);
            }
        }
        float4 rv[NTW];
        uint2 rs[NTW];
        const int64_t bidx = g.rowvec ? m / g.rows_per_batch : 0;
#pragma unroll
        for (int nt = 0; nt < NTW; ++nt) {
            const int64_t n = n_lane + nt * 16;
            const bool okn = n < g.N && !(g.geglu && (nt & 1));
            const int64_t on = g.geglu ? (n_base + wn * (16 * NTW) + nt * 16) / 2 + fc * 4 : n;
            rv[nt] = (g.rowvec && n < g.N) ? *reinterpret_cast<const float4 *>(g.rowvec + bidx * g.ld_rowvec + n) : make_float4(0.f, 0.f, 0.f, 0.f);
            rs[nt] = (g.residual && okn) ? *reinterpret_cast<const uint2 *>((const unsigned char *)g.residual + (m * g.ldr + on) * 2) : make_uint2(0u, 0u);
        }
#pragma unroll
        for (int nt = 0; nt < NTW; ++nt) {
            const int64_t n = n_lane + nt * 16;
            if (n >= g.N) continue;
            if (g.geglu && (nt & 1)) continue;
            float v[4] = {acc[nt][mt][0] + bia[nt].x + rv[nt].x, acc[nt][mt][1] + bia[nt].y + rv[nt].y,
                          acc[nt][mt][2] + bia[nt].z + rv[nt].z, acc[nt][mt][3] + bia[nt].w + rv[nt].w};
            int64_t on = n;
            if (g.geglu) {
                constexpr int NP = NTW - 1;
                const int np = nt + 1 < NTW ? nt + 1 : NP;
                v[0] *= gelu_erf(acc[np][mt][0] + bia[np].x); v[1] *= gelu_erf(acc[np][mt][1] + bia[np].y);
                v[2] *= gelu_erf(acc[np][mt][2] + bia[np].z); v[3] *= gelu_erf(acc[np][mt][3] + bia[np].w);
                on = (n_base + wn * (16 * NTW) + nt * 16) / 2 + fc * 4;
            }
            if (g.act == 1) {
#pragma unroll
                for (int r = 0; r < 4; ++r) v[r] = silu(v[r]);
            } else if (g.act == 2) {
#pragma unroll
                for (int r = 0; r < 4; ++r) v[r] = fminf(fmaxf(v[r] * 0.5f + 0.5f, 0.f), 1.f);
            }
#pragma unroll
            for (int r = 0; r < 4; ++r) v[r] *= g.out_scale;
            if (g.residual) {
                v[0] += T::to_f((unsigned short)(rs[nt].x & 0xffff)); v[1] += T::to_f((unsigned short)(rs[nt].x >> 16));
                v[2] += T::to_f((unsigned short)(rs[nt].y & 0xffff)); v[3] += T::to_f((unsigned short)(rs[nt].y >> 16));
            }
            const bool to_t = g.out_t && on >= g.t_col0;
            const uint2 pk = make_uint2(pack2<T>(v[0], v[1]), pack2<T>(v[2], v[3]));
            if (g.out && !(to_t && g.t_col0 > 0)) {
                if (g.out_f32)
                    *reinterpret_cast<float4 *>((float *)g.out + m * g.ldc + on) = make_float4(v[0], v[1], v[2], v[3]);
                else
                    *reinterpret_cast<uint2 *>((unsigned char *)g.out + (m * g.ldc + on) * 2) = pk;
            }
            if (to_t) {
                const int64_t b = m / g.rows_per_batch, tok = m - b * g.rows_per_batch;
                unsigned short *o = (unsigned short *)g.out_t + b * g.t_batch_stride + tok;
#pragma unroll
                for (int r = 0; r < 4; ++r) o[(on - g.t_col0 + r) * g.ldt] = T::from_f(v[r]);
            }
        }
    }
    }
}


template <class T, int NTW, int MT, int LNV = 0>
__global__ __launch_bounds__(512, 1) void k_gemm8p(const GemmArgs g)
{
    static_assert(LNV == 0 || LNV == 2, "persistent kernel: plain or LayerNorm-folded consumer");
    constexpr int BM = 64 * MT, BN = 32 * NTW, STAGE = BM * 128 + BN * 128, NS = 3;
    constexpr int AG = BM / 8, WG = BN / 8, AI = AG / 8, WI = (WG + 7) / 8;
    static_assert(WG % 8 == 0, "every wave issues the same number of W loads");
    constexpr int GRPW = AI + WI;
    extern __shared__ __attribute__((aligned(16))) unsigned char smem[];
    const int tid = threadIdx.x, lane = tid & 63;
    const int wid = __builtin_amdgcn_readfirstlane(tid >> 6);
    const int wm = wid >> 1, wn = wid & 1;
    const int nbn = (int)((g.N + BN - 1) / BN);
    const int64_t ntiles = ((g.M + BM - 1) / BM) * nbn;
    const int nk = (int)(g.K / BK);
    const unsigned lds0 = (unsigned)(size_t)(__attribute__((address_space(3))) unsigned char *)smem;
    float *srow = reinterpret_cast<float *>(smem + NS * STAGE);
    const int lr = lane >> 3, ls = lane & 7;
    const unsigned char *Ab = (const unsigned char *)g.A, *Wb = (const unsigned char *)g.W;
    auto tile_of = [&](int64_t d, int64_t &m_base, int64_t &n_base) __attribute__((always_inline)) {
        const int64_t xcd = d & 7, qq = ntiles >> 3, rr = ntiles & 7;
        const int64_t bid = (xcd < rr ? xcd * (qq + 1) : rr * (qq + 1) + (xcd - rr) * qq) + (d >> 3);
        int64_t mblk, nblk;
        dng::tile_coords(bid, (int)((g.M + BM - 1) / BM), nbn, g.pw, mblk, nblk);
        m_base = mblk * BM; n_base = nblk * BN;
    };
    int a_off[AI], w_off[WI];
    auto set_offsets = [&](int64_t m_base, int64_t n_base) __attribute__((always_inline)) {
#pragma unroll
        for (int i = 0; i < AI; ++i) {
            const int row = (wid + 8 * i) * 8 + lr;
            const int64_t m = m_base + row;
            a_off[i] = (int)(m < g.M ? m : g.M - 1) * (int)g.lda + (ls ^ ((row >> 1) & 7)) * 8;
        }
#pragma unroll
        for (int i = 0; i < WI; ++i) {
            const int row = (wid + 8 * i) * 8 + lr;
            const int64_t n = n_base + row;
            w_off[i] = (int)(n < g.N ? n : g.N - 1) * (int)g.K + (ls ^ ((row >> 1) & 7)) * 8;
        }
    };
    auto issue_a = [&](int kt, int stage, int i) __attribute__((always_inline)) {
        glds16_s(Ab + (size_t)kt * (BK * 2), (unsigned)(a_off[i] * 2), lds0 + stage * STAGE + (unsigned)((wid + 8 * i) * 1024));
    };
    auto issue_w = [&](int kt, int stage, int i) __attribute__((always_inline)) {
        glds16_s(Wb + (size_t)kt * (BK * 2), (unsigned)(w_off[i] * 2), lds0 + stage * STAGE + (unsigned)(BM * 128 + (wid + 8 * i) * 1024));
    };
    auto issue = [&](int kt, int stage) __attribute__((always_inline)) {
#pragma unroll
        for (int i = 0; i < AI; ++i) issue_a(kt, stage, i);
#pragma unroll
        for (int i = 0; i < WI; ++i) issue_w(kt, stage, i);
    };
    const int fr = lane & 15, fc = lane >> 4;
    const int swz = (fr >> 1) & 7;
    const int fx0 = ((fc ^ swz) << 4), fx1 = (((fc + 4) ^ swz) << 4);
    const int aw0 = BM * 128 + (wn * (16 * NTW) + fr) * 128, aa0 = (wm * (16 * MT) + fr) * 128;
    struct Frag { uint4 w[NTW], a[MT]; };
    auto load_frag = [&](Frag &f, int stage, int ks) __attribute__((always_inline)) {
        const unsigned char *sb = smem + stage * STAGE;
        const int fx = ks ? fx1 : fx0;
#pragma unroll
        for (int t = 0; t < NTW; ++t) f.w[t] = *reinterpret_cast<const uint4 *>(sb + aw0 + fx + t * 2048);
#pragma unroll
        for (int t = 0; t < MT; ++t) f.a[t] = *reinterpret_cast<const uint4 *>(sb + aa0 + fx + t * 2048);
    };
    f32x4 acc[NTW][MT];
    constexpr int NMM = NTW * MT, NPC = AI + WI;
    auto block = [&](const Frag &f, Frag &fn, int st_next, int ks_next, bool load_next, int dma_kt, int dma_stage, auto dma_tag) __attribute__((always_inline)) {
        constexpr bool DMA = decltype(dma_tag)::value;
        static_for<0, NMM>([&](auto m_) __attribute__((always_inline)) {
            constexpr int m = decltype(m_)::value, nt = m / MT, mt = m % MT;
            acc[nt][mt] = T::mfma(f.w[nt], f.a[mt], acc[nt][mt]);
            if constexpr (m == 0) {
                __builtin_amdgcn_sched_barrier(0);
                if (load_next) load_frag(fn, st_next, ks_next);
                __builtin_amdgcn_sched_barrier(0);
            } else if constexpr (DMA && m >= 2) {
                static_for<0, NPC>([&](auto p_) __attribute__((always_inline)) {
                    constexpr int pp = decltype(p_)::value;
                    if constexpr (m == 2 + (pp * (NMM - 3)) / NPC) {
                        __builtin_amdgcn_sched_barrier(0);
                        if constexpr (pp < AI) issue_a(dma_kt, dma_stage, pp); else issue_w(dma_kt, dma_stage, pp - AI);
                        __builtin_amdgcn_sched_barrier(0);
                    }
                });
            }
        });
    };
    auto wait_tiles = [&](auto n_) __attribute__((always_inline)) {
        asm volatile("s_waitcnt vmcnt(%0)" ::"n"(decltype(n_)::value * GRPW) : "memory");
    };

    int64_t d = blockIdx.x, m_base, n_base;
    if (d >= ntiles) return;
    tile_of(d, m_base, n_base);
    set_offsets(m_base, n_base);
    issue(0, 0);
    if (nk > 1) issue(1, 1);
    if (nk > 2) issue(2, 2);
    bool first = true;
    for (;;) {
#pragma unroll
        for (int a = 0; a < NTW; ++a)
#pragma unroll
            for (int b = 0; b < MT; ++b) acc[a][b] = f32x4{0.f, 0.f, 0.f, 0.f};
        if (first) { if (nk > 2) wait_tiles(std::integral_constant<int, 2>{}); else if (nk > 1) wait_tiles(std::integral_constant<int, 1>{}); else wait_tiles(std::integral_constant<int, 0>{}); }
        else asm volatile("s_waitcnt vmcnt(0)" ::: "memory");
        first = false;
        __builtin_amdgcn_s_barrier();
        Frag f0, f1;
        load_frag(f0, 0, 0);
        int st = 0, kt = 0;
        for (; kt + 3 < nk; ++kt) {
            const int st1 = st + 1 == NS ? 0 : st + 1;
            block(f0, f1, st, 1, true, 0, 0, std::false_type{});
            wait_tiles(std::integral_constant<int, 1>{});
            asm volatile("s_waitcnt lgkmcnt(0)" ::: "memory");
            __builtin_amdgcn_s_barrier();
            block(f1, f0, st1, 0, true, kt + 3, st, std::true_type{});
            st = st1;
        }
        for (; kt < nk; ++kt) {
            const int st1 = st + 1 == NS ? 0 : st + 1;
            block(f0, f1, st, 1, true, 0, 0, std::false_type{});
            if (kt + 1 < nk) {
                if (kt + 2 < nk) wait_tiles(std::integral_constant<int, 1>{}); else wait_tiles(std::integral_constant<int, 0>{});
                asm volatile("s_waitcnt lgkmcnt(0)" ::: "memory");
                __builtin_amdgcn_s_barrier();
                block(f1, f0, st1, 0, true, 0, 0, std::false_type{});
            } else {
                block(f1, f0, st1, 0, false, 0, 0, std::false_type{});
            }
            st = st1;
        }
        const int64_t cm = m_base, cn = n_base;
        d += gridDim.x;
        const bool more = d < ntiles;
        asm volatile("s_waitcnt lgkmcnt(0)" ::: "memory");
        __builtin_amdgcn_s_barrier();
        if constexpr (LNV == 2) {
            row_stats_prologue<BM>(g, cm, srow);
            __builtin_amdgcn_s_barrier();
        }
        if (more) {
            tile_of(d, m_base, n_base);
            set_offsets(m_base, n_base);
            issue(0, 0);
            if (nk > 1) issue(1, 1);
            if (nk > 2) issue(2, 2);
        }
        {
            const int64_t n_lane = cn + wn * (16 * NTW) + fc * 4;
            float4 bia[NTW], csm[LNV == 2 ? NTW : 1];
#pragma unroll
            for (int nt = 0; nt < NTW; ++nt) {
                const int64_t n = n_lane + nt * 16;
                bia[nt] = (g.bias && n < g.N) ? *reinterpret_cast<const float4 *>(g.bias + n) : make_float4(0.f, 0.f, 0.f, 0.f);
                if constexpr (LNV == 2) csm[nt] = n < g.N ? *reinterpret_cast<const float4 *>(g.colsum + n) : make_float4(0.f, 0.f, 0.f, 0.f);
            }
            float2 st[LNV == 2 ? MT : 1];
            if constexpr (LNV == 2) {
#pragma unroll
                for (int mt = 0; mt < MT; ++mt) st[mt] = *reinterpret_cast<const float2 *>(srow + 2 * (wm * (16 * MT) + mt * 16 + fr));
            }
#pragma unroll
            for (int mt = 0; mt < MT; ++mt) {
                const int64_t m = cm + wm * (16 * MT) + mt * 16 + fr;
                if (m >= g.M) continue;
                if constexpr (LNV == 2) {
                    const float mean = st[mt].x * g.ln_inv_k, rstd = rsqrtf(fmaxf(st[mt].y * g.ln_inv_k - mean * mean, 0.f) + g.ln_eps);
#pragma unroll
                    for (int nt = 0; nt < NTW; ++nt) {
                        acc[nt][mt][0] = rstd * (acc[nt][mt][0] - mean * csm[nt].x); acc[nt][mt][1] = rstd * (acc[nt][mt][1] - mean * csm[nt].y);
                        acc[nt][mt][2] = rstd * (acc[nt][mt][2] - mean * csm[nt].z); acc[nt][mt][3] = rstd * (acc[nt][mt][3] - mean * csm[nt].w);
                    }
                }
#pragma unroll
                for (int nt = 0; nt < NTW; ++nt) {
                    const int64_t n = n_lane + nt * 16;
                    if (n >= g.N) continue;
                    if (g.geglu && (nt & 1)) continue;
                    float v[4] = {acc[nt][mt][0] + bia[nt].x, acc[nt][mt][1] + bia[nt].y, acc[nt][mt][2] + bia[nt].z, acc[nt][mt][3] + bia[nt].w};
                    int64_t on = n;
                    if (g.geglu) {
                        constexpr int NP = NTW - 1;
                        const int np = nt + 1 < NTW ? nt + 1 : NP;
                        v[0] *= gelu_erf(acc[np][mt][0] + bia[np].x); v[1] *= gelu_erf(acc[np][mt][1] + bia[np].y);
                        v[2] *= gelu_erf(acc[np][mt][2] + bia[np].z); v[3] *= gelu_erf(acc[np][mt][3] + bia[np].w);
                        on = (cn + wn * (16 * NTW) + nt * 16) / 2 + fc * 4;
                    }
                    if (g.act == 1) {
#pragma unroll
                        for (int r = 0; r < 4; ++r) v[r] = silu(v[r]);
                    }
#pragma unroll
                    for (int r = 0; r < 4; ++r) v[r] *= g.out_scale;
                    if (g.residual) {
                        const uint2 rs = *reinterpret_cast<const uint2 *>((const unsigned char *)g.residual + (m * g.ldr + on) * 2);
                        v[0] += T::to_f((unsigned short)(rs.x & 0xffff)); v[1] += T::to_f((unsigned short)(rs.x >> 16));
                        v[2] += T::to_f((unsigned short)(rs.y & 0xffff)); v[3] += T::to_f((unsigned short)(rs.y >> 16));
                    }
                    *reinterpret_cast<uint2 *>((unsigned char *)g.out + (m * g.ldc + on) * 2) = make_uint2(pack2<T>(v[0], v[1]), pack2<T>(v[2], v[3]));
                }
            }
        }
        if (!more) break;
    }
}

template <class T, int NTW, int MT, int LNV = 0>
void launch8p(const GemmArgs &g, int nwg, hipStream_t s)
{
    constexpr size_t lds = 3 * (64 * MT * 128 + 32 * NTW * 128) + (LNV == 2 ? 64 * MT * 8 : 0);
    static_assert(lds <= 160 * 1024, "LDS ring");
    static gc::AttrOnce once;
    gc::ensure_dynamic_lds(once, (const void *)k_gemm8p<T, NTW, MT, LNV>, (int)lds);
    hipLaunchKernelGGL((k_gemm8p<T, NTW, MT, LNV>), dim3(nwg), dim3(512), lds, s, g);
}

typedef __attribute__((ext_vector_type(8))) int i32x8;

template <class T, int MODE, int NTW, int MT, bool FUSE, bool CS = false>
__global__ __launch_bounds__(512, 1) void k_gemm8q(const GemmArgs g)
{
    static_assert(MODE == 2 || MODE == 3, "fp8 path: fast conv (2) and aligned linear (3)");
    constexpr int BM = 64 * MT, BN = 32 * NTW, STAGE = BM * 128 + BN * 128, NS = 3;
    constexpr int AG = BM / 8, WG = BN / 8, AI = AG / 8, WI = (WG + 7) / 8;
    constexpr int BKB = 128;
    extern __shared__ __attribute__((aligned(16))) unsigned char smem[];
    const int tid = threadIdx.x, lane = tid & 63;
    const int wid = __builtin_amdgcn_readfirstlane(tid >> 6);
    const int wm = wid >> 1, wn = wid & 1;
    const int nbn = (int)((g.N + BN - 1) / BN);
    int64_t mblk, nblk;
    int slice;
    wg_tile(g, (int)((g.M + BM - 1) / BM), nbn, mblk, nblk, slice);
    const int64_t m_base = mblk * BM, n_base = nblk * BN;
    const int nk_all = (int)(g.K / BKB);
    const int k0 = g.splits > 1 ? slice * g.tiles_per_split : 0;
    const int nk = g.splits > 1 ? (nk_all - k0 < g.tiles_per_split ? nk_all - k0 : g.tiles_per_split) : nk_all;
    const unsigned lds0 = (unsigned)(size_t)(__attribute__((address_space(3))) unsigned char *)smem;
    float *srow = reinterpret_cast<float *>(smem + NS * STAGE);
    if constexpr (FUSE) {
        if (g.row_stats) row_stats_prologue<BM>(g, m_base, srow);
    }
    static_assert(!(FUSE && CS), "one statistics epilogue at a time");
    float *ctab = reinterpret_cast<float *>(smem + NS * STAGE);
    if constexpr (CS) {
        for (int i = tid; i < 4 * BN; i += 512) ctab[i] = 0.f;
    }
    const int lr = lane >> 3, ls = lane & 7;
    int a_off[AI];
    unsigned a_vm[AI];
    const unsigned char *a_ptr[AI];
#pragma unroll
    for (int i = 0; i < AI; ++i) {
        const int row = (wid + 8 * i) * 8 + lr;
        const int ck = ls ^ ((row >> 1) & 7);
        const int64_t m = m_base + row;
        const bool ok = m < g.M;
        a_vm[i] = 0; a_ptr[i] = (const unsigned char *)g.A; a_off[i] = 0;
        if (MODE == 2) {
            const int mm = ok ? (int)m : 0, hw = g.Ho * g.Wo, b = mm / hw, rem = mm - b * hw, oy = rem / g.Wo;
            const int y0 = oy * g.stride - g.pad, x0 = (rem - oy * g.Wo) * g.stride - g.pad;
            a_ptr[i] = (const unsigned char *)g.A + ((int64_t)(b * g.Hi + y0) * g.Wi + x0) * g.Cin + ck * 16;
            unsigned vm = 0;
#pragma unroll
            for (int tp = 0; tp < 9; ++tp) {
                const int yi = y0 + tp / 3, xi = x0 + tp % 3;
                if (ok && (unsigned)yi < (unsigned)g.Hi && (unsigned)xi < (unsigned)g.Wi) vm |= 1u << tp;
            }
            a_vm[i] = vm;
        } else {
            a_off[i] = (int)(m < g.M ? m : g.M - 1) * (int)g.lda + ck * 16;
        }
    }
    int w_off[WI];
#pragma unroll
    for (int i = 0; i < WI; ++i) {
        const int row = (wid + 8 * i) * 8 + lr;
        const int64_t n = n_base + row;
        w_off[i] = (int)(n < g.N ? n : g.N - 1) * (int)g.K + (ls ^ ((row >> 1) & 7)) * 16;
    }
    const unsigned char *Ab = (const unsigned char *)g.A, *Wb = (const unsigned char *)g.W, *Zp = (const unsigned char *)g.zeros;
    const bool tap_inner = MODE == 2 && g.conv_korder != 0;
    int ld_tap = 0, ld_ci = 0;
    if (MODE == 2) {
        if (tap_inner) { ld_tap = k0 % 9; ld_ci = (k0 / 9) * BKB; }
        else { ld_tap = (k0 * BKB) / g.Cin; ld_ci = (k0 * BKB) % g.Cin; }
    }
    struct TileSrc { int kb, tap, tap_off; unsigned sbase; };
    auto issue_begin = [&](int kt, int stage) __attribute__((always_inline)) -> TileSrc {
        TileSrc t;
        t.kb = (k0 + kt) * BKB; t.tap = 0; t.tap_off = 0;
        if (MODE == 2) {
            t.tap = ld_tap;
            t.kb = __builtin_amdgcn_readfirstlane(ld_tap * g.Cin + ld_ci);
            const int dy = ld_tap / 3, dx = ld_tap - dy * 3;
            t.tap_off = (dy * g.Wi + dx) * g.Cin + ld_ci;
            if (tap_inner) { if (++ld_tap == 9) { ld_tap = 0; ld_ci += BKB; } }
            else { ld_ci += BKB; if (ld_ci >= g.Cin) { ld_ci -= g.Cin; ++ld_tap; } }
        }
        t.sbase = lds0 + stage * STAGE;
        return t;
    };
    auto issue_a = [&](const TileSrc &t, int i) __attribute__((always_inline)) {
        const unsigned dst = t.sbase + (unsigned)((wid + 8 * i) * 1024);
        if (MODE == 3) { glds16_s(Ab + (size_t)t.kb, (unsigned)a_off[i], dst); return; }
        const bool okm = (a_vm[i] >> t.tap) & 1u;
        glds16(okm ? a_ptr[i] + (int64_t)t.tap_off : Zp, dst);
    };
    auto issue_w = [&](const TileSrc &t, int i, bool has) __attribute__((always_inline)) {
        if (has) glds16_s(Wb + (size_t)t.kb, (unsigned)w_off[i], t.sbase + (unsigned)(BM * 128 + (wid + 8 * i) * 1024));
    };
    auto issue = [&](int kt, int stage) __attribute__((always_inline)) {
        const TileSrc t = issue_begin(kt, stage);
#pragma unroll
        for (int i = 0; i < AI; ++i) issue_a(t, i);
#pragma unroll
        for (int i = 0; i < WI; ++i) issue_w(t, i, wid + 8 * i < WG);
    };

    f32x4 acc[NTW][MT];
#pragma unroll
    for (int a = 0; a < NTW; ++a)
#pragma unroll
        for (int b = 0; b < MT; ++b) acc[a][b] = f32x4{0.f, 0.f, 0.f, 0.f};
    const int fr = lane & 15, fc = lane >> 4;
    const int swz = (fr >> 1) & 7;
    const int fx0 = ((fc ^ swz) << 4), fx1 = (((fc + 4) ^ swz) << 4);
    const int aw0 = BM * 128 + (wn * (16 * NTW) + fr) * 128, aa0 = (wm * (16 * MT) + fr) * 128;
    typedef __attribute__((ext_vector_type(4))) int i32x4;
    struct Frag { i32x8 w[NTW], a[MT]; };
    auto ld32 = [&](const unsigned char *p0, const unsigned char *p1) __attribute__((always_inline)) -> i32x8 {
        const i32x4 lo = *reinterpret_cast<const i32x4 *>(p0), hi = *reinterpret_cast<const i32x4 *>(p1);
        return __builtin_shufflevector(lo, hi, 0, 1, 2, 3, 4, 5, 6, 7);
    };
    auto load_frag = [&](Frag &f, int stage) __attribute__((always_inline)) {
        const unsigned char *sb = smem + stage * STAGE;
#pragma unroll
        for (int t = 0; t < NTW; ++t) f.w[t] = ld32(sb + aw0 + fx0 + t * 2048, sb + aw0 + fx1 + t * 2048);
#pragma unroll
        for (int t = 0; t < MT; ++t) f.a[t] = ld32(sb + aa0 + fx0 + t * 2048, sb + aa0 + fx1 + t * 2048);
    };
    int sw[NTW];
#pragma unroll
    for (int t = 0; t < NTW; ++t) {
        const int64_t n = n_base + wn * (16 * NTW) + t * 16 + fr;
        sw[t] = g.w_scale[n < g.N ? n : g.N - 1];
    }
    asm volatile("s_waitcnt vmcnt(0)" ::: "memory");
#pragma unroll
    for (int t = 0; t < NTW; ++t) asm volatile("" : "+v"(sw[t]));
    const int sa = g.a_scale;
    constexpr int NMM = NTW * MT, NPC = AI + WI;
    auto block = [&](const Frag &f, Frag &fn, int st_next, bool load_next, const TileSrc &t, auto dma_tag, auto w3_tag) __attribute__((always_inline)) {
        constexpr bool DMA = decltype(dma_tag)::value, W3 = decltype(w3_tag)::value;
        static_for<0, NMM>([&](auto m_) __attribute__((always_inline)) {
            constexpr int m = decltype(m_)::value, nt = m / MT, mt = m % MT;
            acc[nt][mt] = __builtin_amdgcn_mfma_scale_f32_16x16x128_f8f6f4(f.w[nt], f.a[mt], acc[nt][mt], 0, 0, 0, sw[nt], 0, sa);
            if constexpr (m == 0) {
                __builtin_amdgcn_sched_barrier(0);
                if (load_next) load_frag(fn, st_next);
                __builtin_amdgcn_sched_barrier(0);
            } else if constexpr (DMA && m >= 2) {
                static_for<0, NPC>([&](auto p_) __attribute__((always_inline)) {
                    constexpr int pp = decltype(p_)::value;
                    if constexpr (m == 2 + (pp * (NMM - 3)) / NPC) {
                        __builtin_amdgcn_sched_barrier(0);
                        if constexpr (pp < AI) issue_a(t, pp); else issue_w(t, pp - AI, (pp - AI) < WI - 1 || W3 || WG % 8 == 0);
                        __builtin_amdgcn_sched_barrier(0);
                    }
                });
            }
        });
    };
    const bool w3 = (wid + 8 * (WI - 1)) < WG;
    Frag f0, f1;
    const TileSrc tnone = {0, 0, 0, 0u};
    auto run = [&](auto w3_tag) __attribute__((always_inline)) {
        constexpr bool W3 = decltype(w3_tag)::value;
        constexpr int GRPW = AI + ((W3 || WG % 8 == 0) ? WI : WI - 1);
        auto wait_tiles = [&](auto n_) __attribute__((always_inline)) {
            asm volatile("s_waitcnt vmcnt(%0)" ::"n"(decltype(n_)::value * GRPW) : "memory");
        };
        issue(0, 0);
        if (nk > 1) issue(1, 1);
        if (nk > 2) issue(2, 2);
        if (nk > 2) wait_tiles(std::integral_constant<int, 2>{}); else if (nk > 1) wait_tiles(std::integral_constant<int, 1>{}); else wait_tiles(std::integral_constant<int, 0>{});
        __builtin_amdgcn_s_barrier();
        load_frag(f0, 0);
        int st = 0, kt = 0;
        auto step = [&](Frag &fc_, Frag &fn_) __attribute__((always_inline)) {
            const int st1 = st + 1 == NS ? 0 : st + 1;
            if (kt + 3 < nk) {
                wait_tiles(std::integral_constant<int, 1>{});
                asm volatile("s_waitcnt lgkmcnt(0)" ::: "memory");
                __builtin_amdgcn_s_barrier();
                const TileSrc t = issue_begin(kt + 3, st);
                block(fc_, fn_, st1, true, t, std::true_type{}, w3_tag);
            } else if (kt + 1 < nk) {
                if (kt + 2 < nk) wait_tiles(std::integral_constant<int, 1>{}); else wait_tiles(std::integral_constant<int, 0>{});
                asm volatile("s_waitcnt lgkmcnt(0)" ::: "memory");
                __builtin_amdgcn_s_barrier();
                block(fc_, fn_, st1, true, tnone, std::false_type{}, w3_tag);
            } else {
                block(fc_, fn_, st1, false, tnone, std::false_type{}, w3_tag);
            }
            st = st1; ++kt;
        };
        while (kt < nk) {
            step(f0, f1);
            if (kt < nk) step(f1, f0);
        }
    };
    if (w3) run(std::true_type{}); else run(std::false_type{});
    if constexpr (FUSE) {
        wave_epilogue<T, NTW, MT, 512>(g, acc, m_base, m_base + wm * (16 * MT), n_base + wn * (16 * NTW), lane, smem, g.row_stats ? srow : nullptr, slice);
        return;
    }
    const int64_t n_lane = n_base + wn * (16 * NTW) + fc * 4;
    if (g.splits > 1) {
#pragma unroll
        for (int mt = 0; mt < MT; ++mt) {
            const int64_t m = m_base + wm * (16 * MT) + mt * 16 + fr;
            if (m >= g.M) continue;
#pragma unroll
            for (int nt = 0; nt < NTW; ++nt) {
                const int64_t n = n_lane + nt * 16;
                if (n < g.N)
                    *reinterpret_cast<float4 *>(g.ws + ((int64_t)slice * g.M + m) * g.N + n) =
                        make_float4(acc[nt][mt][0], acc[nt][mt][1], acc[nt][mt][2], acc[nt][mt][3]);
            }
        }
        return;
    }
    if constexpr (CS) {
        const unsigned char *zp = (const unsigned char *)g.zeros;
        const bool has_b = g.bias != nullptr, has_rv = g.rowvec != nullptr, has_res = g.residual != nullptr;
        const float *biasp = has_b ? g.bias : reinterpret_cast<const float *>(zp);
        const float *rvp = has_rv ? g.rowvec : reinterpret_cast<const float *>(zp);
        const unsigned char *resp = has_res ? (const unsigned char *)g.residual : zp;
        const int64_t bA = m_base / g.rows_per_batch, b_last = (g.M - 1) / g.rows_per_batch;
        const int64_t bB = bA + 1 < b_last ? bA + 1 : b_last;
        const int64_t m_rv = (bA + 1) * g.rows_per_batch;
        float4 bia[NTW], rvA[NTW], rvB[NTW];
        uint2 rs[MT][NTW];
#pragma unroll
        for (int nt = 0; nt < NTW; ++nt) {
            const int64_t n = n_lane + nt * 16, nc = n < g.N ? n : g.N - 4;
            bia[nt] = *reinterpret_cast<const float4 *>(biasp + (has_b ? nc : 0));
            rvA[nt] = *reinterpret_cast<const float4 *>(rvp + (has_rv ? bA * g.ld_rowvec + nc : 0));
            rvB[nt] = *reinterpret_cast<const float4 *>(rvp + (has_rv ? bB * g.ld_rowvec + nc : 0));
        }
#pragma unroll
        for (int mt = 0; mt < MT; ++mt) {
            const int64_t m = m_base + wm * (16 * MT) + mt * 16 + fr, mc = m < g.M ? m : g.M - 1;
#pragma unroll
            for (int nt = 0; nt < NTW; ++nt) {
                const int64_t n = n_lane + nt * 16, nc = n < g.N ? n : g.N - 4;
                rs[mt][nt] = *reinterpret_cast<const uint2 *>(resp + (has_res ? (mc * g.ldr + nc) * 2 : 0));
            }
        }
        uint2 pks[MT][NTW];
#pragma unroll
        for (int mt = 0; mt < MT; ++mt) {
            const int64_t m = m_base + wm * (16 * MT) + mt * 16 + fr;
            const bool second = m >= m_rv;
#pragma unroll
            for (int nt = 0; nt < NTW; ++nt) {
                const int64_t n = n_lane + nt * 16;
                const float4 rv = second ? rvB[nt] : rvA[nt];
                float v[4] = {acc[nt][mt][0] + bia[nt].x + rv.x, acc[nt][mt][1] + bia[nt].y + rv.y,
                              acc[nt][mt][2] + bia[nt].z + rv.z, acc[nt][mt][3] + bia[nt].w + rv.w};
#pragma unroll
                for (int r = 0; r < 4; ++r) v[r] *= g.out_scale;
                v[0] += T::to_f((unsigned short)(rs[mt][nt].x & 0xffff)); v[1] += T::to_f((unsigned short)(rs[mt][nt].x >> 16));
                v[2] += T::to_f((unsigned short)(rs[mt][nt].y & 0xffff)); v[3] += T::to_f((unsigned short)(rs[mt][nt].y >> 16));
                const uint2 pk = make_uint2(pack2<T>(v[0], v[1]), pack2<T>(v[2], v[3]));
                const bool ok = m < g.M && n < g.N;
                if (ok) *reinterpret_cast<uint2 *>((unsigned char *)g.out + (m * g.ldc + n) * 2) = pk;
                pks[mt][nt] = ok ? pk : make_uint2(0u, 0u);
            }
        }
        {
            const int64_t m_split = (m_base / g.rows_per_batch + 1) * g.rows_per_batch;
            const int64_t m_end = m_base + BM < g.M ? m_base + BM : g.M;
            const int npass = m_split < m_end ? 2 : 1;
    #pragma unroll 1
            for (int pass = 0; pass < npass; ++pass) {
                float cs[NTW][4], cq[NTW][4];
    #pragma unroll
                for (int nt = 0; nt < NTW; ++nt)
    #pragma unroll
                    for (int r = 0; r < 4; ++r) { cs[nt][r] = 0.f; cq[nt][r] = 0.f; }
    #pragma unroll
                for (int mt = 0; mt < MT; ++mt) {
                    const int64_t m_tile = m_base + wm * (16 * MT) + mt * 16;
                    const float wgt = ((m_tile >= m_split ? 1 : 0) == pass) ? 1.f : 0.f;
    #pragma unroll
                    for (int nt = 0; nt < NTW; ++nt) {
                        const uint2 pk = pks[mt][nt];
                        const float t0 = wgt != 0.f ? T::to_f((unsigned short)(pk.x & 0xffff)) : 0.f, t1 = wgt != 0.f ? T::to_f((unsigned short)(pk.x >> 16)) : 0.f;
                        const float t2 = wgt != 0.f ? T::to_f((unsigned short)(pk.y & 0xffff)) : 0.f, t3 = wgt != 0.f ? T::to_f((unsigned short)(pk.y >> 16)) : 0.f;
                        cs[nt][0] += t0; cq[nt][0] += t0 * t0; cs[nt][1] += t1; cq[nt][1] += t1 * t1;
                        cs[nt][2] += t2; cq[nt][2] += t2 * t2; cs[nt][3] += t3; cq[nt][3] += t3 * t3;
                    }
                }
                float *tb = ctab + (pass * BN + wn * (16 * NTW) + fc * 4) * 2;
    #pragma unroll
                for (int nt = 0; nt < NTW; ++nt)
    #pragma unroll
                    for (int r = 0; r < 4; ++r) {
                        const float sa = row16_sum(cs[nt][r]), sb = row16_sum(cq[nt][r]);
                        if (fr == 0) {
                            __hip_atomic_fetch_add(tb + (nt * 16 + r) * 2, sa, __ATOMIC_RELAXED, __HIP_MEMORY_SCOPE_WORKGROUP);
                            __hip_atomic_fetch_add(tb + (nt * 16 + r) * 2 + 1, sb, __ATOMIC_RELAXED, __HIP_MEMORY_SCOPE_WORKGROUP);
                        }
                    }
            }
            asm volatile("s_waitcnt lgkmcnt(0)" ::: "memory");
            __builtin_amdgcn_s_barrier();
            const int64_t b0 = m_base / g.rows_per_batch;
            const int cpg = g.gn_cpg, G = (int)(g.N / cpg);
            const int n_hi = (int)(n_base + BN < g.N ? n_base + BN : g.N);
            const int g_first = (int)n_base / cpg, ng = (n_hi - 1) / cpg - g_first + 1;
            for (int i = tid; i < 2 * ng; i += 512) {
                const int slot = i >= ng ? 1 : 0, gg = g_first + i - slot * ng;
                if (slot == 1 && !(m_split < m_end)) continue;
                const int c_lo = gg * cpg > (int)n_base ? gg * cpg : (int)n_base, c_hi = (gg + 1) * cpg < n_hi ? (gg + 1) * cpg : n_hi;
                float s1 = 0.f, s2 = 0.f;
                for (int c = c_lo; c < c_hi; ++c) { const float2 t = *reinterpret_cast<const float2 *>(ctab + (slot * BN + c - (int)n_base) * 2); s1 += t.x; s2 += t.y; }
                const int64_t b = b0 + slot;
                const int64_t slab = mblk - (b * g.rows_per_batch) / BM;
                const int half = gg * cpg < (int)n_base ? 1 : 0;
                *reinterpret_cast<float2 *>(g.chan_parts + ((((b * g.cp_nslab + slab) * G + gg) * 2 + half) * 2)) = make_float2(s1, s2);
            }
        }
        return;
    }
    float4 bia[NTW];
#pragma unroll
    for (int nt = 0; nt < NTW; ++nt) {
        const int64_t n = n_lane + nt * 16;
        bia[nt] = (g.bias && n < g.N) ? *reinterpret_cast<const float4 *>(g.bias + n) : make_float4(0.f, 0.f, 0.f, 0.f);
    }
#pragma unroll
    for (int mt = 0; mt < MT; ++mt) {
        const int64_t m = m_base + wm * (16 * MT) + mt * 16 + fr;
        if (m >= g.M) continue;
        float4 rv[NTW];
        uint2 rs[NTW];
        const int64_t bidx = g.rowvec ? m / g.rows_per_batch : 0;
#pragma unroll
        for (int nt = 0; nt < NTW; ++nt) {
            const int64_t n = n_lane + nt * 16;
            const bool okn = n < g.N && !(g.geglu && (nt & 1));
            const int64_t on = g.geglu ? (n_base + wn * (16 * NTW) + nt * 16) / 2 + fc * 4 : n;
            rv[nt] = (g.rowvec && n < g.N) ? *reinterpret_cast<const float4 *>(g.rowvec + bidx * g.ld_rowvec + n) : make_float4(0.f, 0.f, 0.f, 0.f);
            rs[nt] = (g.residual && okn) ? *reinterpret_cast<const uint2 *>((const unsigned char *)g.residual + (m * g.ldr + on) * 2) : make_uint2(0u, 0u);
        }
#pragma unroll
        for (int nt = 0; nt < NTW; ++nt) {
            const int64_t n = n_lane + nt * 16;
            if (n >= g.N) continue;
            if (g.geglu && (nt & 1)) continue;
            float v[4] = {acc[nt][mt][0] + bia[nt].x + rv[nt].x, acc[nt][mt][1] + bia[nt].y + rv[nt].y,
                          acc[nt][mt][2] + bia[nt].z + rv[nt].z, acc[nt][mt][3] + bia[nt].w + rv[nt].w};
            int64_t on = n;
            if (g.geglu) {
                constexpr int NP = NTW - 1;
                const int np = nt + 1 < NTW ? nt + 1 : NP;
                v[0] *= gelu_erf(acc[np][mt][0] + bia[np].x); v[1] *= gelu_erf(acc[np][mt][1] + bia[np].y);
                v[2] *= gelu_erf(acc[np][mt][2] + bia[np].z); v[3] *= gelu_erf(acc[np][mt][3] + bia[np].w);
                on = (n_base + wn * (16 * NTW) + nt * 16) / 2 + fc * 4;
            }
            if (g.act == 1) {
#pragma unroll
                for (int r = 0; r < 4; ++r) v[r] = silu(v[r]);
            } else if (g.act == 2) {
#pragma unroll
                for (int r = 0; r < 4; ++r) v[r] = fminf(fmaxf(v[r] * 0.5f + 0.5f, 0.f), 1.f);
            }
#pragma unroll
            for (int r = 0; r < 4; ++r) v[r] *= g.out_scale;
            if (g.residual) {
                v[0] += T::to_f((unsigned short)(rs[nt].x & 0xffff)); v[1] += T::to_f((unsigned short)(rs[nt].x >> 16));
                v[2] += T::to_f((unsigned short)(rs[nt].y & 0xffff)); v[3] += T::to_f((unsigned short)(rs[nt].y >> 16));
            }
            const bool to_t = g.out_t && on >= g.t_col0;
            if (g.out_fp8) {
                const float q0 = fminf(fmaxf(v[0] * g.out_qscale, -448.f), 448.f), q1 = fminf(fmaxf(v[1] * g.out_qscale, -448.f), 448.f);
                const float q2 = fminf(fmaxf(v[2] * g.out_qscale, -448.f), 448.f), q3 = fminf(fmaxf(v[3] * g.out_qscale, -448.f), 448.f);
                int w8 = 0;
                w8 = __builtin_amdgcn_cvt_pk_fp8_f32(q0, q1, w8, false); w8 = __builtin_amdgcn_cvt_pk_fp8_f32(q2, q3, w8, true);
                *reinterpret_cast<int *>((unsigned char *)g.out + m * g.ldc + on) = w8;
            } else if (g.out && !(to_t && g.t_col0 > 0)) {
                if (g.out_f32)
                    *reinterpret_cast<float4 *>((float *)g.out + m * g.ldc + on) = make_float4(v[0], v[1], v[2], v[3]);
                else
                    *reinterpret_cast<uint2 *>((unsigned char *)g.out + (m * g.ldc + on) * 2) = make_uint2(pack2<T>(v[0], v[1]), pack2<T>(v[2], v[3]));
            }
            if (to_t) {
                const int64_t b = m / g.rows_per_batch, tok = m - b * g.rows_per_batch;
                unsigned short *o = (unsigned short *)g.out_t + b * g.t_batch_stride + tok;
#pragma unroll
                for (int r = 0; r < 4; ++r) o[(on - g.t_col0 + r) * g.ldt] = T::from_f(v[r]);
            }
        }
    }
}

constexpr int ZC = 8;
template <class T>
__global__ __launch_bounds__(256) void k_splitk_epilogue_plain(const GemmArgs g)
{
    const int64_t nq = g.N / 4;
    for (int64_t q = (int64_t)blockIdx.x * 256 + threadIdx.x; q < g.M * nq; q += (int64_t)gridDim.x * 256) {
        const int64_t m = q / nq, n = (q - m * nq) * 4;
        float v[4] = {0.f, 0.f, 0.f, 0.f};
        const uint2 rpre = g.residual ? *reinterpret_cast<const uint2 *>((const unsigned char *)g.residual + (m * g.ldr + n) * 2) : make_uint2(0u, 0u);
        for (int z0 = 0; z0 < g.splits; z0 += ZC) {
            float4 a[ZC];
#pragma unroll
            for (int u = 0; u < ZC; ++u)
                if (z0 + u < g.splits) a[u] = *reinterpret_cast<const float4 *>(g.ws + ((int64_t)(z0 + u) * g.M + m) * g.N + n);
#pragma unroll
            for (int u = 0; u < ZC; ++u)
                if (z0 + u < g.splits) { v[0] += a[u].x; v[1] += a[u].y; v[2] += a[u].z; v[3] += a[u].w; }
        }
        float gate[4] = {0.f, 0.f, 0.f, 0.f};
        epilogue_store<T>(g, m, n, n, v, gate, &rpre);
    }
}

template <class T>
__global__ __launch_bounds__(256) void k_splitk_epilogue(const GemmArgs g)
{
    __shared__ float red[GS_MAXG * 2];
    constexpr int RPB = 16;
    const int64_t nq = g.N / 4;
    const int cl = threadIdx.x & 63, rl = threadIdx.x >> 6;
    const int64_t cq = (int64_t)blockIdx.x * 64 + cl;
    const int64_t m0 = (int64_t)blockIdx.y * RPB;
    const bool okc = cq < nq;
    const int64_t n = (okc ? cq : 0) * 4;
    if (g.out_group_stats) {
        if (threadIdx.x < GS_MAXG * 2) red[threadIdx.x] = 0.f;
        __syncthreads();
    }
    float v[4][4];
#pragma unroll
    for (int i = 0; i < 4; ++i) { v[i][0] = 0.f; v[i][1] = 0.f; v[i][2] = 0.f; v[i][3] = 0.f; }
    if (okc) {
        for (int z0 = 0; z0 < g.splits; z0 += ZC / 2) {
            float4 a[ZC / 2][4];
#pragma unroll
            for (int u = 0; u < ZC / 2; ++u)
#pragma unroll
                for (int i = 0; i < 4; ++i) {
                    const int64_t m = m0 + rl + 4 * i;
                    if (z0 + u < g.splits && m < g.M) a[u][i] = *reinterpret_cast<const float4 *>(g.ws + ((int64_t)(z0 + u) * g.M + m) * g.N + n);
                }
#pragma unroll
            for (int u = 0; u < ZC / 2; ++u)
#pragma unroll
                for (int i = 0; i < 4; ++i) {
                    const int64_t m = m0 + rl + 4 * i;
                    if (z0 + u < g.splits && m < g.M) { v[i][0] += a[u][i].x; v[i][1] += a[u][i].y; v[i][2] += a[u][i].z; v[i][3] += a[u][i].w; }
                }
        }
    }
    float cs[8] = {0.f, 0.f, 0.f, 0.f, 0.f, 0.f, 0.f, 0.f};
#pragma unroll
    for (int i = 0; i < 4; ++i) {
        const int64_t m = m0 + rl + 4 * i;
        if (m >= g.M) break;
        if (okc) {
            float gate[4] = {0.f, 0.f, 0.f, 0.f};
            epilogue_store<T>(g, m, n, n, v[i], gate);
        }
        if (g.out_row_stats) {
            const float a = wave_sum_f(okc ? (v[i][0] + v[i][1]) + (v[i][2] + v[i][3]) : 0.f);
            const float b = wave_sum_f(okc ? (v[i][0] * v[i][0] + v[i][1] * v[i][1]) + (v[i][2] * v[i][2] + v[i][3] * v[i][3]) : 0.f);
            if (cl == 0) *reinterpret_cast<float2 *>(g.out_row_stats + ((int64_t)blockIdx.x * g.M + m) * 2) = make_float2(a, b);
        }
        if (okc) {
#pragma unroll
            for (int r = 0; r < 4; ++r) { cs[2 * r] += v[i][r]; cs[2 * r + 1] += v[i][r] * v[i][r]; }
        }
    }
    if (g.out_group_stats) {
        if (okc) {
#pragma unroll
            for (int r = 0; r < 4; ++r) {
                const int gi = (int)(n + r) / g.gn_cpg;
                __hip_atomic_fetch_add(red + 2 * gi, cs[2 * r], __ATOMIC_RELAXED, __HIP_MEMORY_SCOPE_WORKGROUP);
                __hip_atomic_fetch_add(red + 2 * gi + 1, cs[2 * r + 1], __ATOMIC_RELAXED, __HIP_MEMORY_SCOPE_WORKGROUP);
            }
        }
        __syncthreads();
        if (threadIdx.x < GS_MAXG * 2) {
            const float t = red[threadIdx.x];
            if (t != 0.f) unsafeAtomicAdd(g.out_group_stats + (m0 / g.rows_per_batch) * g.gn_groups * 2 + threadIdx.x, t);
        }
    }
}


constexpr int CS_RB = 32;
template <class T>
__global__ __launch_bounds__(256) void k_splitk_epilogue_cs(const GemmArgs g)
{
    __shared__ float red[16][16][8];
    constexpr int RPT = CS_RB / 16;
    const int64_t nq = g.N / 4;
    const int cl = threadIdx.x & 15, rl = threadIdx.x >> 4;
    const int64_t cq4 = (int64_t)blockIdx.x * 16 + cl;
    const int64_t m0 = (int64_t)blockIdx.y * CS_RB;
    const bool okc = cq4 < nq;
    const int64_t n = (okc ? cq4 : 0) * 4;
    float cs[8] = {0.f, 0.f, 0.f, 0.f, 0.f, 0.f, 0.f, 0.f};
    float v[RPT][4];
#pragma unroll
    for (int i = 0; i < RPT; ++i) { v[i][0] = 0.f; v[i][1] = 0.f; v[i][2] = 0.f; v[i][3] = 0.f; }
    if (okc) {
        uint2 rpre[RPT];
#pragma unroll
        for (int i = 0; i < RPT; ++i) {
            const int64_t m = m0 + rl + 16 * i;
            rpre[i] = (g.residual && m < g.M) ? *reinterpret_cast<const uint2 *>((const unsigned char *)g.residual + (m * g.ldr + n) * 2) : make_uint2(0u, 0u);
        }
        for (int z0 = 0; z0 < g.splits; z0 += ZC) {
            float4 a[ZC][RPT];
#pragma unroll
            for (int u = 0; u < ZC; ++u)
#pragma unroll
                for (int i = 0; i < RPT; ++i) {
                    const int64_t m = m0 + rl + 16 * i;
                    if (z0 + u < g.splits && m < g.M) a[u][i] = *reinterpret_cast<const float4 *>(g.ws + ((int64_t)(z0 + u) * g.M + m) * g.N + n);
                }
#pragma unroll
            for (int u = 0; u < ZC; ++u)
#pragma unroll
                for (int i = 0; i < RPT; ++i) {
                    const int64_t m = m0 + rl + 16 * i;
                    if (z0 + u < g.splits && m < g.M) { v[i][0] += a[u][i].x; v[i][1] += a[u][i].y; v[i][2] += a[u][i].z; v[i][3] += a[u][i].w; }
                }
        }
#pragma unroll
        for (int i = 0; i < RPT; ++i) {
            const int64_t m = m0 + rl + 16 * i;
            if (m >= g.M) break;
            float gate[4] = {0.f, 0.f, 0.f, 0.f};
            epilogue_store<T>(g, m, n, n, v[i], gate, &rpre[i]);
#pragma unroll
            for (int r = 0; r < 4; ++r) { cs[2 * r] += v[i][r]; cs[2 * r + 1] += v[i][r] * v[i][r]; }
        }
    }
#pragma unroll
    for (int j = 0; j < 8; ++j) red[rl][cl][j] = cs[j];
    __syncthreads();
    __shared__ float chs[64][2];
    if (threadIdx.x < 128) {
        const int c2 = threadIdx.x >> 3, j = threadIdx.x & 7;
        float o = 0.f;
#pragma unroll
        for (int r = 0; r < 16; ++r) o += red[r][c2][j];
        chs[c2 * 4 + (j >> 1)][j & 1] = o;
    }
    __syncthreads();
    if (m0 < g.M) {
        const int cpg = g.gn_cpg, G = (int)(g.N / cpg);
        const int n_base = (int)blockIdx.x * 64, n_hi = n_base + 64 < (int)g.N ? n_base + 64 : (int)g.N;
        const int g_first = n_base / cpg, ng = (n_hi - 1) / cpg - g_first + 1;
        if ((int)threadIdx.x < ng) {
            const int gg = g_first + threadIdx.x;
            const int c_lo = gg * cpg > n_base ? gg * cpg : n_base, c_hi = (gg + 1) * cpg < n_hi ? (gg + 1) * cpg : n_hi;
            float s1 = 0.f, s2 = 0.f;
            for (int c = c_lo; c < c_hi; ++c) { s1 += chs[c - n_base][0]; s2 += chs[c - n_base][1]; }
            const int64_t b = m0 / g.rows_per_batch, slab = (m0 - b * g.rows_per_batch) / CS_RB;
            const int half = gg * cpg < n_base ? 1 : 0;
            *reinterpret_cast<float2 *>(g.chan_parts + ((((b * g.cp_nslab + slab) * G + gg) * 2 + half) * 2)) = make_float2(s1, s2);
        }
    }
}


inline bool fuse_of(const GemmArgs &g) { return g.row_stats || g.out_row_stats || g.out_group_stats; }

template <class F>
void with_wave_tile(int ntw, int mt, F &&f)
{
    const auto with_mt = [&](auto ntw_) {
        if (mt == 4) f(ntw_, std::integral_constant<int, 4>{}); else if (mt == 3) f(ntw_, std::integral_constant<int, 3>{}); else f(ntw_, std::integral_constant<int, 2>{});
    };
    if (ntw == 5) with_mt(std::integral_constant<int, 5>{}); else with_mt(std::integral_constant<int, 4>{});
}

template <class T, int MODE, int NTW, bool FUSE>
void launch4(const GemmArgs &g, dim3 grid, hipStream_t s)
{
    constexpr size_t lds = 2 * (BM * 128 + 32 * NTW * 128);
    static gc::AttrOnce once;
    gc::ensure_dynamic_lds(once, (const void *)k_gemm<T, MODE, NTW, FUSE>, (int)lds);
    hipLaunchKernelGGL((k_gemm<T, MODE, NTW, FUSE>), grid, dim3(NT), lds, s, g);
}

template <class T, int MODE, int NTW, int MT, bool FUSE, bool CS = false, bool LEAN = false, int LNV = 0>
void launch8(const GemmArgs &g, dim3 grid, hipStream_t s)
{
    constexpr size_t lds = 3 * (64 * MT * 128 + 32 * NTW * 128) + ((FUSE || LNV >= 2) ? 64 * MT * 8 : 0) + (CS ? 32 * NTW * 16 : 0);
    static_assert(lds <= 160 * 1024, "LDS ring");
    static gc::AttrOnce once;
    gc::ensure_dynamic_lds(once, (const void *)k_gemm8<T, MODE, NTW, MT, FUSE, CS, LEAN, LNV>, (int)lds);
    hipLaunchKernelGGL((k_gemm8<T, MODE, NTW, MT, FUSE, CS, LEAN, LNV>), grid, dim3(512), lds, s, g);
}

inline bool ln_lean_producer_of(const GemmArgs &g, int mode, int splits)
{
    return g.out_row_stats && !g.row_stats && !g.out_group_stats && !g.chan_parts && splits == 1 && mode == 0 && g.K % 64 == 0 && !g.geglu &&
           g.act == 0 && !g.out_f32 && !g.out_t && g.out && g.N >= 4 && (!g.rowvec || g.rows_per_batch >= 256);
}
inline bool ln_lean_consumer_of(const GemmArgs &g, int mode, int splits)
{
    return g.row_stats && !g.out_row_stats && !g.out_group_stats && !g.chan_parts && splits == 1 && mode == 0 && g.K % 64 == 0 && g.N >= 4;
}
template <class T, int NTW, int MT>
void dispatch8ln_m(const GemmArgs &g, int lnv, bool lean, dim3 grid, hipStream_t s)
{
    if (lnv == 3) { if constexpr (NTW == 5) launch8<T, 3, 5, MT, false, false, false, 3>(g, grid, s); return; }
    if (lnv == 1) launch8<T, 3, NTW, MT, false, false, true, 1>(g, grid, s);
    else if (lean) launch8<T, 3, NTW, MT, false, false, true, 2>(g, grid, s);
    else launch8<T, 3, NTW, MT, false, false, false, 2>(g, grid, s);
}
template <class T>
void dispatch8ln(const GemmArgs &g, int lnv, bool lean, int ntw, int mt, dim3 grid, hipStream_t s)
{
    if (lnv == 2 && g.persist > 0 && ntw == 4 && mt == 4) { launch8p<T, 4, 4, 2>(g, g.persist, s); return; }
    if (mt == 1 && ntw == 4) { dispatch8ln_m<T, 4, 1>(g, lnv, lean, grid, s); return; }
    with_wave_tile(ntw, mt, [&](auto ntw_, auto mt_) { dispatch8ln_m<T, decltype(ntw_)::value, decltype(mt_)::value>(g, lnv, lean, grid, s); });
}

inline bool lean_of(const GemmArgs &g, int mode)
{
    return !g.geglu && g.act == 0 && !g.out_f32 && !g.out_t && g.out && mode != 1 && (mode != 0 || g.K % 64 == 0) && g.N >= 4 &&
           (!g.rowvec || g.rows_per_batch >= 256);
}
template <class T, int NTW, int MT>
void dispatch8lean_m(const GemmArgs &g, int mode, dim3 grid, hipStream_t s)
{
    if (mode == 0) launch8<T, 3, NTW, MT, false, false, true>(g, grid, s);
    else if (g.ups) launch8<T, 4, NTW, MT, false, false, true>(g, grid, s);
    else launch8<T, 2, NTW, MT, false, false, true>(g, grid, s);
}
template <class T>
void dispatch8lean(const GemmArgs &g, int mode, int ntw, int mt, dim3 grid, hipStream_t s)
{
    if (mt == 1 && ntw == 4 && mode == 0) { launch8<T, 3, 4, 1, false, false, true>(g, grid, s); return; }
    with_wave_tile(ntw, mt, [&](auto ntw_, auto mt_) { dispatch8lean_m<T, decltype(ntw_)::value, decltype(mt_)::value>(g, mode, grid, s); });
}

template <class T, int NTW, int MT>
void dispatch8cs_m(const GemmArgs &g, int mode, dim3 grid, hipStream_t s)
{
    if (mode == 0) launch8<T, 3, NTW, MT, false, true>(g, grid, s);
    else if (mode == 1) launch8<T, 1, NTW, MT, false, true>(g, grid, s);
    else launch8<T, 2, NTW, MT, false, true>(g, grid, s);
}
template <class T>
void dispatch8cs(const GemmArgs &g, int mode, int ntw, int mt, dim3 grid, hipStream_t s)
{
    with_wave_tile(ntw, mt, [&](auto ntw_, auto mt_) { dispatch8cs_m<T, decltype(ntw_)::value, decltype(mt_)::value>(g, mode, grid, s); });
}

template <class T, int NTW, int MT, bool FUSE>
void dispatch8m(const GemmArgs &g, int mode, dim3 grid, hipStream_t s)
{
    if constexpr (FUSE) {
        if (mode == 0) launch8<T, 3, NTW, MT, true>(g, grid, s);
        else if (mode == 1) launch8<T, 1, NTW, MT, true>(g, grid, s);
        else launch8<T, 2, NTW, MT, true>(g, grid, s);
    } else {
        if (mode == 0) { if (g.K % 64 == 0) launch8<T, 3, NTW, MT, false>(g, grid, s); else launch8<T, 0, NTW, MT, false>(g, grid, s); }
        else if (mode == 1) launch8<T, 1, NTW, MT, false>(g, grid, s);
        else if (g.ups) launch8<T, 4, NTW, MT, false>(g, grid, s); else launch8<T, 2, NTW, MT, false>(g, grid, s);
    }
}
template <class T, bool FUSE>
void dispatch8(const GemmArgs &g, int mode, int ntw, int mt, dim3 grid, hipStream_t s)
{
    if constexpr (!FUSE) {
        if (mt == 1 && ntw == 4 && mode == 0 && g.K % 64 == 0) { launch8<T, 3, 4, 1, false>(g, grid, s); return; }
        if (g.persist > 0 && ntw == 4 && mt == 4 && mode == 0) { launch8p<T, 4, 4>(g, g.persist, s); return; }
    }
    with_wave_tile(ntw, mt, [&](auto ntw_, auto mt_) { dispatch8m<T, decltype(ntw_)::value, decltype(mt_)::value, FUSE>(g, mode, grid, s); });
}

template <class T, bool FUSE>
void dispatch4(const GemmArgs &g, int mode, int ntw, dim3 grid, hipStream_t s)
{
    if (ntw == 5) {
        if (mode == 0) launch4<T, 0, 5, FUSE>(g, grid, s); else if (mode == 1) launch4<T, 1, 5, FUSE>(g, grid, s); else launch4<T, 2, 5, FUSE>(g, grid, s);
    } else {
        if (mode == 0) launch4<T, 0, 4, FUSE>(g, grid, s); else if (mode == 1) launch4<T, 1, 4, FUSE>(g, grid, s); else launch4<T, 2, 4, FUSE>(g, grid, s);
    }
}

}

using dng::GemmArgs;
void dn_gemm_launch_plain(const GemmArgs &g, int dtype, int mode, int ntw, int mt8, dim3 grid, hipStream_t s);
void dn_gemm_launch_fuse(const GemmArgs &g, int dtype, int mode, int ntw, int mt8, dim3 grid, hipStream_t s);
void dn_gemm_launch_fp8(const GemmArgs &g, int dtype, int mode, int ntw, int mt, dim3 grid, hipStream_t s);
void dn_gemm_launch_splitk_epilogue(const GemmArgs &g, int dtype, hipStream_t s);
void dn_gemm_launch_cs(const GemmArgs &g, int dtype, int mode, int ntw, int mt8, dim3 grid, hipStream_t s);
void dn_gemm_launch_splitk_epilogue_cs(const GemmArgs &g, int dtype, hipStream_t s);
void dn_gemm_launch_lean(const GemmArgs &g, int dtype, int mode, int ntw, int mt8, dim3 grid, hipStream_t s);
void dn_gemm_launch_ln(const GemmArgs &g, int dtype, int lnv, bool lean, int ntw, int mt8, dim3 grid, hipStream_t s);
```

Measured before the change: 10.83.

## Unify persistent GEMM walk into main body and extend it to convs and lean epilogues

Folds the separate persistent GEMM kernel into the main gemm8 body behind a PERSIST template flag. Each workgroup walks tiles in XCD order and prefetches the next tile's LDS ring before running the current epilogue. Persistence now also covers stride-1 3x3 convs, the lean and channel-stats epilogues, more tile shapes (mt8 >= 2) and much larger K. The aim is to cut launch and tail costs and overlap epilogue work with the next tile's loads across more of the denoiser. In exchange it adds code complexity, register pressure at occupancy 1, and an abort path for the unsupported 160x256 tile.

```diff
diff --git a/gaussctrl_amd/csrc/dn_gemm.hip b/gaussctrl_amd/csrc/dn_gemm.hip
--- a/gaussctrl_amd/csrc/dn_gemm.hip
+++ b/gaussctrl_amd/csrc/dn_gemm.hip
@@ -249,6 +249,7 @@
 }
 
 namespace {
+constexpr int64_t PERSIST_MAX_K = 9 * 1920;
 struct Route { Sel sel; int lnk, persist; };
 void route(const gc_gemm_desc *d, const GemmVariant &v, Route *r)
 {
@@ -258,10 +259,12 @@
     const bool fuse = d->ln_row_stats || d->out_row_stats || d->out_group_stats;
     r->lnk = (sel.mt8 && sel.splits == 1) ? ln_lean_kind(d, v) : 0;
     r->persist = 0;
-    if (sel.mt8 == 4 && sel.ntw == 4 && sel.mode == 0 && sel.splits == 1 && d->K % 64 == 0 && d->K <= 64 * 24 && (!fuse || r->lnk == 2) && !d->out_chan_parts &&
-        !d->rowvec && !d->out_t && !d->out_f32 && d->out && d->act != 2 && !v.no_persist) {
-        const int64_t tiles = ((d->M + 255) / 256) * ((d->N + 32 * sel.ntw - 1) / (32 * sel.ntw));
-        if (tiles > 256) r->persist = 256;
+    const bool lin = sel.mode == 0 && d->K % 64 == 0 && !d->out_chan_parts;
+    const bool conv = sel.mode == 2 && d->stride == 1 && !d->upsample && lean_of(*d, sel.mode) && (d->out_chan_parts || !v.full_epilogue);
+    const bool fits = !(sel.ntw == 5 && sel.mt8 == 4);
+    if (!v.no_persist && fits && sel.mt8 >= 2 && sel.splits == 1 && (lin || conv) && (!fuse || r->lnk == 1 || r->lnk == 2) && !d->out_f32 && d->out && d->act != 2) {
+        const int64_t tiles = ((d->M + 64 * sel.mt8 - 1) / (64 * sel.mt8)) * ((d->N + 32 * sel.ntw - 1) / (32 * sel.ntw));
+        if (tiles > 256 && d->K <= PERSIST_MAX_K) r->persist = 256;
     }
 }
 }
@@ -393,10 +396,10 @@
         const int64_t nbm8 = (d->M + 64 * sel.mt8 - 1) / (64 * sel.mt8);
         const dim3 grid8((unsigned)(nbm8 * nbn), (unsigned)sel.splits);
         g.pw = pw_of(d, v, nbm8, nbn, g.persist ? 8 * 32 : nbm8 * nbn * sel.splits, sel.mt8 == 1 ? 64 : 32, 64 * sel.mt8, bn);
-        if (lnk) dn_gemm_launch_ln(g, d->dtype, lnk, lean_of(g, sel.mode) && g.persist == 0, sel.ntw, sel.mt8, grid8, s);
+        if (lnk) dn_gemm_launch_ln(g, d->dtype, lnk, lean_of(g, sel.mode), sel.ntw, sel.mt8, grid8, s);
         else if (fuse_of(g)) dn_gemm_launch_fuse(g, d->dtype, sel.mode, sel.ntw, sel.mt8 < 2 ? 2 : sel.mt8, grid8, s);
         else if (g.chan_parts && sel.splits == 1) dn_gemm_launch_cs(g, d->dtype, sel.mode, sel.ntw, sel.mt8, grid8, s);
-        else if (lean_of(g, sel.mode) && g.persist == 0 && !v.full_epilogue) dn_gemm_launch_lean(g, d->dtype, sel.mode, sel.ntw, sel.mt8, grid8, s);
+        else if (lean_of(g, sel.mode) && !v.full_epilogue) dn_gemm_launch_lean(g, d->dtype, sel.mode, sel.ntw, sel.mt8, grid8, s);
         else dn_gemm_launch_plain(g, d->dtype, sel.mode, sel.ntw, sel.mt8, grid8, s);
     } else {
         const int64_t nbm = (d->M + BM - 1) / BM;
diff --git a/gaussctrl_amd/csrc/dn_gemm_kernels.h b/gaussctrl_amd/csrc/dn_gemm_kernels.h
--- a/gaussctrl_amd/csrc/dn_gemm_kernels.h
+++ b/gaussctrl_amd/csrc/dn_gemm_kernels.h
@@ -41,11 +41,15 @@
     const int64_t w = (nbn - p * pw) < pw ? (nbn - p * pw) : pw;
     mblk = within / w; nblk = p * pw + within % w;
 }
+__device__ __forceinline__ int64_t xcd_order(int64_t lin, int64_t total)
+{
+    const int64_t xcd = lin & 7, qq = total >> 3, rr = total & 7;
+    return (xcd < rr ? xcd * (qq + 1) : rr * (qq + 1) + (xcd - rr) * qq) + (lin >> 3);
+}
 __device__ __forceinline__ void wg_tile(const GemmArgs &g, int nbm, int nbn, int64_t &mblk, int64_t &nblk, int &slice)
 {
     const int64_t tiles = gridDim.x, total = tiles * gridDim.y, lin = blockIdx.x + tiles * blockIdx.y;
-    const int64_t xcd = lin & 7, qq = total >> 3, rr = total & 7;
-    const int64_t L = (xcd < rr ? xcd * (qq + 1) : rr * (qq + 1) + (xcd - rr) * qq) + (lin >> 3);
+    const int64_t L = xcd_order(lin, total);
     slice = (int)(L / tiles);
     tile_coords(L - (int64_t)slice * tiles, nbm, nbn, g.pw, mblk, nblk);
 }
@@ -647,9 +651,10 @@
     asm volatile("s_mov_b32 m0, %2\n\ts_nop 0\n\tglobal_load_lds_dwordx4 %0, %1" :: "v"(voff), "s"(sbase), "s"(lds_dst) : "memory");
 }
 
-template <class T, int MODE, int NTW, int MT, bool FUSE, bool CS = false, bool LEAN_ = false, int LNV = 0>
-__global__ __launch_bounds__(512, MT <= 2 ? 2 : 1) void k_gemm8(const GemmArgs g)
-{
+template <class T, int MODE, int NTW, int MT, bool FUSE, bool CS, bool LEAN_, int LNV, bool PERSIST>
+__device__ __forceinline__ void gemm8_body(const GemmArgs &g)
+{
+    static_assert(!PERSIST || (!FUSE && LNV != 3 && (MODE == 2 || MODE == 3)), "persistent walk: fast conv / K % 64 == 0 linear on the non-FUSE epilogues");
     static_assert(!(FUSE && CS), "one statistics epilogue at a time");
     static_assert(LNV == 0 || (!FUSE && !CS && MODE == 3), "lean LayerNorm fold: K % 64 == 0 linears on the non-FUSE epilogues");
     static_assert(LNV != 1 || LEAN_, "row partials come from the lean epilogue");
@@ -667,85 +672,97 @@
     const int tid = threadIdx.x, lane = tid & 63;
     const int wid = __builtin_amdgcn_readfirstlane(tid >> 6);
     const int wm = wid >> 1, wn = wid & 1;
-    const int nbn = (int)((g.N + BN - 1) / BN);
-    int64_t mblk, nblk;
-    int slice;
-    wg_tile(g, (int)((g.M + BM - 1) / BM), nbn, mblk, nblk, slice);
-    const int64_t m_base = mblk * BM, n_base = nblk * BN;
+    const int nbm = (int)((g.M + BM - 1) / BM), nbn = (int)((g.N + BN - 1) / BN);
+    int64_t mblk, nblk, d = blockIdx.x;
+    const int64_t ntiles = (int64_t)nbm * nbn;
+    int slice = 0;
+    if constexpr (PERSIST) {
+        if (d >= ntiles) return;
+        dng::tile_coords(dng::xcd_order(d, ntiles), nbm, nbn, g.pw, mblk, nblk);
+    } else {
+        wg_tile(g, nbm, nbn, mblk, nblk, slice);
+    }
+    int64_t m_base, n_base, wset;
     const int nk_all = (int)((g.K + BK - 1) / BK);
     const int kt0 = slice * g.tiles_per_split;
     const int nk = min(nk_all, kt0 + g.tiles_per_split) - kt0;
     const unsigned lds0 = (unsigned)(size_t)(__attribute__((address_space(3))) unsigned char *)smem;
     float *srow = reinterpret_cast<float *>(smem + NS * STAGE);
-    if constexpr (FUSE) {
-        if (g.row_stats && g.splits == 1) row_stats_prologue<BM>(g, m_base, srow);
-    }
     float *ctab = reinterpret_cast<float *>(smem + NS * STAGE);
-    if constexpr (CS) {
-        for (int i = tid; i < 4 * BN; i += 512) ctab[i] = 0.f;
-    }
 
     const int lr = lane >> 3, ls = lane & 7;
     int a_off[AI], a_y[AI], a_x[AI], a_ck[AI];
     bool a_ok[AI];
-#pragma unroll
-    for (int i = 0; i < AI; ++i) {
-        const int row = (wid + 8 * i) * 8 + lr;
-        a_ck[i] = ls ^ ((row >> 1) & 7);
-        const int64_t m = m_base + row;
-        a_ok[i] = m < g.M;
-        const int mm = a_ok[i] ? (int)m : 0;
-        if (MODE == 1 || CONVF) {
-            const int hw = g.Ho * g.Wo;
-            const int b = mm / hw;
-            const int rem = mm - b * hw;
-            const int oy = rem / g.Wo;
-            a_y[i] = oy * g.stride - g.pad; a_x[i] = (rem - oy * g.Wo) * g.stride - g.pad;
-            a_off[i] = b * g.Hi * g.Wi * g.Cin + (CONVF ? a_ck[i] * 8 : 0);
-            if (MODE == 2) a_off[i] += (a_y[i] * g.Wi + a_x[i]) * g.Cin;
-        } else {
-            a_off[i] = mm * (int)g.lda + a_ck[i] * 8;
-            if (MODE == 3) a_off[i] = (int)(m < g.M ? m : g.M - 1) * (int)g.lda + a_ck[i] * 8;
-            a_y[i] = a_x[i] = 0;
-        }
-    }
     int w_off[WI], w_ck[WI];
     bool w_ok[WI];
-#pragma unroll
-    for (int i = 0; i < WI; ++i) {
-        const int grp = wid + 8 * i;
-        const int row = grp * 8 + lr;
-        w_ck[i] = ls ^ ((row >> 1) & 7);
-        const int64_t n = n_base + row;
-        w_ok[i] = grp < WG && n < g.N;
-        w_off[i] = (w_ok[i] ? (int)n : 0) * (int)g.K + w_ck[i] * 8;
-        if (MODE == 3) w_off[i] = (int)(n < g.N ? n : g.N - 1) * (int)g.K + w_ck[i] * 8;
-    }
     const bool ups = CONVF ? UPS : (g.ups != 0);
     const int Hin = ups ? g.Hi * 2 : g.Hi, Win = ups ? g.Wi * 2 : g.Wi;
     const unsigned char *a_ptr[AI];
     unsigned a_vm[AI];
-    if (MODE == 2) {
-#pragma unroll
-        for (int i = 0; i < AI; ++i) {
-            a_ptr[i] = (const unsigned char *)g.A + (int64_t)a_off[i] * 2;
-            unsigned vm = 0;
-#pragma unroll
-            for (int tp = 0; tp < 9; ++tp) {
-                const int yi = a_y[i] + tp / 3, xi = a_x[i] + tp % 3;
-                if (a_ok[i] && (unsigned)yi < (unsigned)Hin && (unsigned)xi < (unsigned)Win) vm |= 1u << tp;
-            }
-            a_vm[i] = vm;
-        }
-    }
-    const int64_t wset = (LNV != 0 && g.w_set_rows > 0) ? m_base / g.w_set_rows : 0;
-    const unsigned char *Ab = (const unsigned char *)g.A, *Wb = (const unsigned char *)g.W + (LNV != 0 ? wset * g.w_set_stride * 2 : 0);
+    const unsigned char *Ab = (const unsigned char *)g.A, *Wb = (const unsigned char *)g.W;
     const unsigned char *Zp = (const unsigned char *)g.zeros;
     const bool tap_inner = CONVF && g.conv_korder != 0;
     int ld_tap = 0, ld_ci = 0;
-    if (CONVF && kt0 > 0) {
-        if (tap_inner) { ld_tap = kt0 % 9; ld_ci = (kt0 / 9) * BK; }
-        else { ld_tap = (kt0 * BK) / g.Cin; ld_ci = kt0 * BK - ld_tap * g.Cin; }
+    auto set_tile = [&]() __attribute__((always_inline)) {
+        m_base = mblk * BM; n_base = nblk * BN;
+#pragma unroll
+        for (int i = 0; i < AI; ++i) {
+            const int row = (wid + 8 * i) * 8 + lr;
+            a_ck[i] = ls ^ ((row >> 1) & 7);
+            const int64_t m = m_base + row;
+            a_ok[i] = m < g.M;
+            const int mm = a_ok[i] ? (int)m : 0;
+            if (MODE == 1 || CONVF) {
+                const int hw = g.Ho * g.Wo;
+                const int b = mm / hw;
+                const int rem = mm - b * hw;
+                const int oy = rem / g.Wo;
+                a_y[i] = oy * g.stride - g.pad; a_x[i] = (rem - oy * g.Wo) * g.stride - g.pad;
+                a_off[i] = b * g.Hi * g.Wi * g.Cin + (CONVF ? a_ck[i] * 8 : 0);
+                if (MODE == 2) a_off[i] += (a_y[i] * g.Wi + a_x[i]) * g.Cin;
+            } else {
+                a_off[i] = mm * (int)g.lda + a_ck[i] * 8;
+                if (MODE == 3) a_off[i] = (int)(m < g.M ? m : g.M - 1) * (int)g.lda + a_ck[i] * 8;
+                a_y[i] = a_x[i] = 0;
+            }
+        }
+#pragma unroll
+        for (int i = 0; i < WI; ++i) {
+            const int grp = wid + 8 * i;
+            const int row = grp * 8 + lr;
+            w_ck[i] = ls ^ ((row >> 1) & 7);
+            const int64_t n = n_base + row;
+            w_ok[i] = grp < WG && n < g.N;
+            w_off[i] = (w_ok[i] ? (int)n : 0) * (int)g.K + w_ck[i] * 8;
+            if (MODE == 3) w_off[i] = (int)(n < g.N ? n : g.N - 1) * (int)g.K + w_ck[i] * 8;
+        }
+        if (MODE == 2) {
+#pragma unroll
+            for (int i = 0; i < AI; ++i) {
+                a_ptr[i] = (const unsigned char *)g.A + (int64_t)a_off[i] * 2;
+                unsigned vm = 0;
+#pragma unroll
+                for (int tp = 0; tp < 9; ++tp) {
+                    const int yi = a_y[i] + tp / 3, xi = a_x[i] + tp % 3;
+                    if (a_ok[i] && (unsigned)yi < (unsigned)Hin && (unsigned)xi < (unsigned)Win) vm |= 1u << tp;
+                }
+                a_vm[i] = vm;
+            }
+        }
+        wset = (LNV != 0 && g.w_set_rows > 0) ? __builtin_amdgcn_readfirstlane((int)(m_base / g.w_set_rows)) : 0;
+        Wb = (const unsigned char *)g.W + (LNV != 0 ? wset * g.w_set_stride * 2 : 0);
+        ld_tap = 0; ld_ci = 0;
+        if (CONVF && kt0 > 0) {
+            if (tap_inner) { ld_tap = kt0 % 9; ld_ci = (kt0 / 9) * BK; }
+            else { ld_tap = (kt0 * BK) / g.Cin; ld_ci = kt0 * BK - ld_tap * g.Cin; }
+        }
+    };
+    set_tile();
+    if constexpr (FUSE) {
+        if (g.row_stats && g.splits == 1) row_stats_prologue<BM>(g, m_base, srow);
+    }
+    if constexpr (CS && !PERSIST) {
+        for (int i = tid; i < 4 * BN; i += 512) ctab[i] = 0.f;
     }
 
     struct TileSrc { int kb, dy_u, dx_u, tap_off, tap; unsigned sbase; };
@@ -813,10 +830,6 @@
     };
 
     f32x4 acc[NTW][MT];
-#pragma unroll
-    for (int a = 0; a < NTW; ++a)
-#pragma unroll
-        for (int b = 0; b < MT; ++b) acc[a][b] = f32x4{0.f, 0.f, 0.f, 0.f};
     const int fr = lane & 15, fc = lane >> 4;
     const int swz = (fr >> 1) & 7;
     const int fx0 = ((fc ^ swz) << 4), fx1 = (((fc + 4) ^ swz) << 4);
@@ -856,19 +869,24 @@
     const bool w3 = (wid + 8 * (WI - 1)) < WG;
     Frag f0, f1;
     const TileSrc tnone = {0, 0, 0, 0, 0, 0u};
-    auto run = [&](auto w3_tag) __attribute__((always_inline)) {
+    auto fill_ring = [&]() __attribute__((always_inline)) {
+        issue(0, 0);
+        if (nk > 1) issue(1, 1);
+        if (nk > 2) issue(2, 2);
+    };
+    auto run = [&](auto w3_tag, bool first) __attribute__((always_inline)) {
         constexpr bool W3 = decltype(w3_tag)::value;
         constexpr int GRPW = AI + ((W3 || WG % 8 == 0) ? WI : WI - 1);
         static_assert(2 * GRPW < 64, "vmcnt range");
         auto wait_tiles = [&](auto n_) __attribute__((always_inline)) {
             asm volatile("s_waitcnt vmcnt(%0)" ::"n"(decltype(n_)::value * GRPW) : "memory");
         };
-        issue(0, 0);
-        if (nk > 1) issue(1, 1);
-        if (nk > 2) issue(2, 2);
-        if constexpr (LNIN) row_stats_prologue<BM>(g, m_base, srow);
-        if (nk > 2) wait_tiles(std::integral_constant<int, 2>{}); else if (nk > 1) wait_tiles(std::integral_constant<int, 1>{}); else wait_tiles(std::integral_constant<int, 0>{});
+        if (!PERSIST || first) { if (nk > 2) wait_tiles(std::integral_constant<int, 2>{}); else if (nk > 1) wait_tiles(std::integral_constant<int, 1>{}); else wait_tiles(std::integral_constant<int, 0>{}); }
+        else asm volatile("s_waitcnt vmcnt(0)" ::: "memory");
         __builtin_amdgcn_s_barrier();
+        if constexpr (PERSIST && CS) {
+            for (int i = tid; i < 4 * BN; i += 512) ctab[i] = 0.f;
+        }
         load_frag(f0, 0, 0);
         int st = 0, kt = 0;
         for (; kt + 3 < nk; ++kt) {
@@ -895,8 +913,7 @@
             st = st1;
         }
     };
-    if (w3) run(std::true_type{}); else run(std::false_type{});
-
+    auto epilogue = [&](const int64_t m_base, const int64_t n_base, const int64_t mblk, const int64_t wset) __attribute__((always_inline)) {
     if constexpr (FUSE) {
         wave_epilogue<T, NTW, MT, 512>(g, acc, m_base, m_base + wm * (16 * MT), n_base + wn * (16 * NTW), lane, smem,
                                        (g.row_stats && g.splits == 1) ? srow : nullptr, slice);
@@ -1174,227 +1191,66 @@
         }
     }
     }
-}
-
-
-template <class T, int NTW, int MT, int LNV = 0>
-__global__ __launch_bounds__(512, 1) void k_gemm8p(const GemmArgs g)
-{
-    static_assert(LNV == 0 || LNV == 2, "persistent kernel: plain or LayerNorm-folded consumer");
-    constexpr int BM = 64 * MT, BN = 32 * NTW, STAGE = BM * 128 + BN * 128, NS = 3;
-    constexpr int AG = BM / 8, WG = BN / 8, AI = AG / 8, WI = (WG + 7) / 8;
-    static_assert(WG % 8 == 0, "every wave issues the same number of W loads");
-    constexpr int GRPW = AI + WI;
-    extern __shared__ __attribute__((aligned(16))) unsigned char smem[];
-    const int tid = threadIdx.x, lane = tid & 63;
-    const int wid = __builtin_amdgcn_readfirstlane(tid >> 6);
-    const int wm = wid >> 1, wn = wid & 1;
-    const int nbn = (int)((g.N + BN - 1) / BN);
-    const int64_t ntiles = ((g.M + BM - 1) / BM) * nbn;
-    const int nk = (int)(g.K / BK);
-    const unsigned lds0 = (unsigned)(size_t)(__attribute__((address_space(3))) unsigned char *)smem;
-    float *srow = reinterpret_cast<float *>(smem + NS * STAGE);
-    const int lr = lane >> 3, ls = lane & 7;
-    const unsigned char *Ab = (const unsigned char *)g.A, *Wb = (const unsigned char *)g.W;
-    auto tile_of = [&](int64_t d, int64_t &m_base, int64_t &n_base) __attribute__((always_inline)) {
-        const int64_t xcd = d & 7, qq = ntiles >> 3, rr = ntiles & 7;
-        const int64_t bid = (xcd < rr ? xcd * (qq + 1) : rr * (qq + 1) + (xcd - rr) * qq) + (d >> 3);
-        int64_t mblk, nblk;
-        dng::tile_coords(bid, (int)((g.M + BM - 1) / BM), nbn, g.pw, mblk, nblk);
-        m_base = mblk * BM; n_base = nblk * BN;
-    };
-    int a_off[AI], w_off[WI];
-    auto set_offsets = [&](int64_t m_base, int64_t n_base) __attribute__((always_inline)) {
-#pragma unroll
-        for (int i = 0; i < AI; ++i) {
-            const int row = (wid + 8 * i) * 8 + lr;
-            const int64_t m = m_base + row;
-            a_off[i] = (int)(m < g.M ? m : g.M - 1) * (int)g.lda + (ls ^ ((row >> 1) & 7)) * 8;
-        }
-#pragma unroll
-        for (int i = 0; i < WI; ++i) {
-            const int row = (wid + 8 * i) * 8 + lr;
-            const int64_t n = n_base + row;
-            w_off[i] = (int)(n < g.N ? n : g.N - 1) * (int)g.K + (ls ^ ((row >> 1) & 7)) * 8;
-        }
-    };
-    auto issue_a = [&](int kt, int stage, int i) __attribute__((always_inline)) {
-        glds16_s(Ab + (size_t)kt * (BK * 2), (unsigned)(a_off[i] * 2), lds0 + stage * STAGE + (unsigned)((wid + 8 * i) * 1024));
-    };
-    auto issue_w = [&](int kt, int stage, int i) __attribute__((always_inline)) {
-        glds16_s(Wb + (size_t)kt * (BK * 2), (unsigned)(w_off[i] * 2), lds0 + stage * STAGE + (unsigned)(BM * 128 + (wid + 8 * i) * 1024));
-    };
-    auto issue = [&](int kt, int stage) __attribute__((always_inline)) {
-#pragma unroll
-        for (int i = 0; i < AI; ++i) issue_a(kt, stage, i);
-#pragma unroll
-        for (int i = 0; i < WI; ++i) issue_w(kt, stage, i);
-    };
-    const int fr = lane & 15, fc = lane >> 4;
-    const int swz = (fr >> 1) & 7;
-    const int fx0 = ((fc ^ swz) << 4), fx1 = (((fc + 4) ^ swz) << 4);
-    const int aw0 = BM * 128 + (wn * (16 * NTW) + fr) * 128, aa0 = (wm * (16 * MT) + fr) * 128;
-    struct Frag { uint4 w[NTW], a[MT]; };
-    auto load_frag = [&](Frag &f, int stage, int ks) __attribute__((always_inline)) {
-        const unsigned char *sb = smem + stage * STAGE;
-        const int fx = ks ? fx1 : fx0;
-#pragma unroll
-        for (int t = 0; t < NTW; ++t) f.w[t] = *reinterpret_cast<const uint4 *>(sb + aw0 + fx + t * 2048);
-#pragma unroll
-        for (int t = 0; t < MT; ++t) f.a[t] = *reinterpret_cast<const uint4 *>(sb + aa0 + fx + t * 2048);
-    };
-    f32x4 acc[NTW][MT];
-    constexpr int NMM = NTW * MT, NPC = AI + WI;
-    auto block = [&](const Frag &f, Frag &fn, int st_next, int ks_next, bool load_next, int dma_kt, int dma_stage, auto dma_tag) __attribute__((always_inline)) {
-        constexpr bool DMA = decltype(dma_tag)::value;
-        static_for<0, NMM>([&](auto m_) __attribute__((always_inline)) {
-            constexpr int m = decltype(m_)::value, nt = m / MT, mt = m % MT;
-            acc[nt][mt] = T::mfma(f.w[nt], f.a[mt], acc[nt][mt]);
-            if constexpr (m == 0) {
-                __builtin_amdgcn_sched_barrier(0);
-                if (load_next) load_frag(fn, st_next, ks_next);
-                __builtin_amdgcn_sched_barrier(0);
-            } else if constexpr (DMA && m >= 2) {
-                static_for<0, NPC>([&](auto p_) __attribute__((always_inline)) {
-                    constexpr int pp = decltype(p_)::value;
-                    if constexpr (m == 2 + (pp * (NMM - 3)) / NPC) {
-                        __builtin_amdgcn_sched_barrier(0);
-                        if constexpr (pp < AI) issue_a(dma_kt, dma_stage, pp); else issue_w(dma_kt, dma_stage, pp - AI);
-                        __builtin_amdgcn_sched_barrier(0);
-                    }
-                });
-            }
-        });
-    };
-    auto wait_tiles = [&](auto n_) __attribute__((always_inline)) {
-        asm volatile("s_waitcnt vmcnt(%0)" ::"n"(decltype(n_)::value * GRPW) : "memory");
-    };
-
-    int64_t d = blockIdx.x, m_base, n_base;
-    if (d >= ntiles) return;
-    tile_of(d, m_base, n_base);
-    set_offsets(m_base, n_base);
-    issue(0, 0);
-    if (nk > 1) issue(1, 1);
-    if (nk > 2) issue(2, 2);
-    bool first = true;
-    for (;;) {
+    };
+
+    fill_ring();
+    for (bool first = true;; first = false) {
 #pragma unroll
         for (int a = 0; a < NTW; ++a)
 #pragma unroll
             for (int b = 0; b < MT; ++b) acc[a][b] = f32x4{0.f, 0.f, 0.f, 0.f};
-        if (first) { if (nk > 2) wait_tiles(std::integral_constant<int, 2>{}); else if (nk > 1) wait_tiles(std::integral_constant<int, 1>{}); else wait_tiles(std::integral_constant<int, 0>{}); }
-        else asm volatile("s_waitcnt vmcnt(0)" ::: "memory");
-        first = false;
-        __builtin_amdgcn_s_barrier();
-        Frag f0, f1;
-        load_frag(f0, 0, 0);
-        int st = 0, kt = 0;
-        for (; kt + 3 < nk; ++kt) {
-            const int st1 = st + 1 == NS ? 0 : st + 1;
-            block(f0, f1, st, 1, true, 0, 0, std::false_type{});
-            wait_tiles(std::integral_constant<int, 1>{});
+        if constexpr (LNIN && !PERSIST) row_stats_prologue<BM>(g, m_base, srow);
+        if (WG % 8 == 0 || w3) run(std::true_type{}, first); else run(std::false_type{}, first);
+        if constexpr (!PERSIST) {
+            epilogue(m_base, n_base, mblk, wset);
+            return;
+        } else {
+            const int64_t cm = m_base, cn = n_base, cmblk = mblk, cwset = wset;
+            d += gridDim.x;
+            const bool more = d < ntiles;
             asm volatile("s_waitcnt lgkmcnt(0)" ::: "memory");
             __builtin_amdgcn_s_barrier();
-            block(f1, f0, st1, 0, true, kt + 3, st, std::true_type{});
-            st = st1;
-        }
-        for (; kt < nk; ++kt) {
-            const int st1 = st + 1 == NS ? 0 : st + 1;
-            block(f0, f1, st, 1, true, 0, 0, std::false_type{});
-            if (kt + 1 < nk) {
-                if (kt + 2 < nk) wait_tiles(std::integral_constant<int, 1>{}); else wait_tiles(std::integral_constant<int, 0>{});
-                asm volatile("s_waitcnt lgkmcnt(0)" ::: "memory");
+            if constexpr (LNIN) {
+                row_stats_prologue<BM>(g, cm, srow);
                 __builtin_amdgcn_s_barrier();
-                block(f1, f0, st1, 0, true, 0, 0, std::false_type{});
-            } else {
-                block(f1, f0, st1, 0, false, 0, 0, std::false_type{});
-            }
-            st = st1;
-        }
-        const int64_t cm = m_base, cn = n_base;
-        d += gridDim.x;
-        const bool more = d < ntiles;
-        asm volatile("s_waitcnt lgkmcnt(0)" ::: "memory");
-        __builtin_amdgcn_s_barrier();
-        if constexpr (LNV == 2) {
-            row_stats_prologue<BM>(g, cm, srow);
-            __builtin_amdgcn_s_barrier();
-        }
-        if (more) {
-            tile_of(d, m_base, n_base);
-            set_offsets(m_base, n_base);
-            issue(0, 0);
-            if (nk > 1) issue(1, 1);
-            if (nk > 2) issue(2, 2);
-        }
-        {
-            const int64_t n_lane = cn + wn * (16 * NTW) + fc * 4;
-            float4 bia[NTW], csm[LNV == 2 ? NTW : 1];
-#pragma unroll
-            for (int nt = 0; nt < NTW; ++nt) {
-                const int64_t n = n_lane + nt * 16;
-                bia[nt] = (g.bias && n < g.N) ? *reinterpret_cast<const float4 *>(g.bias + n) : make_float4(0.f, 0.f, 0.f, 0.f);
-                if constexpr (LNV == 2) csm[nt] = n < g.N ? *reinterpret_cast<const float4 *>(g.colsum + n) : make_float4(0.f, 0.f, 0.f, 0.f);
-            }
-            float2 st[LNV == 2 ? MT : 1];
-            if constexpr (LNV == 2) {
-#pragma unroll
-                for (int mt = 0; mt < MT; ++mt) st[mt] = *reinterpret_cast<const float2 *>(srow + 2 * (wm * (16 * MT) + mt * 16 + fr));
-            }
-#pragma unroll
-            for (int mt = 0; mt < MT; ++mt) {
-                const int64_t m = cm + wm * (16 * MT) + mt * 16 + fr;
-                if (m >= g.M) continue;
-                if constexpr (LNV == 2) {
-                    const float mean = st[mt].x * g.ln_inv_k, rstd = rsqrtf(fmaxf(st[mt].y * g.ln_inv_k - mean * mean, 0.f) + g.ln_eps);
-#pragma unroll
-                    for (int nt = 0; nt < NTW; ++nt) {
-                        acc[nt][mt][0] = rstd * (acc[nt][mt][0] - mean * csm[nt].x); acc[nt][mt][1] = rstd * (acc[nt][mt][1] - mean * csm[nt].y);
-                        acc[nt][mt][2] = rstd * (acc[nt][mt][2] - mean * csm[nt].z); acc[nt][mt][3] = rstd * (acc[nt][mt][3] - mean * csm[nt].w);
-                    }
-                }
-#pragma unroll
-                for (int nt = 0; nt < NTW; ++nt) {
-                    const int64_t n = n_lane + nt * 16;
-                    if (n >= g.N) continue;
-                    if (g.geglu && (nt & 1)) continue;
-                    float v[4] = {acc[nt][mt][0] + bia[nt].x, acc[nt][mt][1] + bia[nt].y, acc[nt][mt][2] + bia[nt].z, acc[nt][mt][3] + bia[nt].w};
-                    int64_t on = n;
-                    if (g.geglu) {
-                        constexpr int NP = NTW - 1;
-                        const int np = nt + 1 < NTW ? nt + 1 : NP;
-                        v[0] *= gelu_erf(acc[np][mt][0] + bia[np].x); v[1] *= gelu_erf(acc[np][mt][1] + bia[np].y);
-                        v[2] *= gelu_erf(acc[np][mt][2] + bia[np].z); v[3] *= gelu_erf(acc[np][mt][3] + bia[np].w);
-                        on = (cn + wn * (16 * NTW) + nt * 16) / 2 + fc * 4;
-                    }
-                    if (g.act == 1) {
-#pragma unroll
-                        for (int r = 0; r < 4; ++r) v[r] = silu(v[r]);
-                    }
-#pragma unroll
-                    for (int r = 0; r < 4; ++r) v[r] *= g.out_scale;
-                    if (g.residual) {
-                        const uint2 rs = *reinterpret_cast<const uint2 *>((const unsigned char *)g.residual + (m * g.ldr + on) * 2);
-                        v[0] += T::to_f((unsigned short)(rs.x & 0xffff)); v[1] += T::to_f((unsigned short)(rs.x >> 16));
-                        v[2] += T::to_f((unsigned short)(rs.y & 0xffff)); v[3] += T::to_f((unsigned short)(rs.y >> 16));
-                    }
-                    *reinterpret_cast<uint2 *>((unsigned char *)g.out + (m * g.ldc + on) * 2) = make_uint2(pack2<T>(v[0], v[1]), pack2<T>(v[2], v[3]));
-                }
-            }
-        }
-        if (!more) break;
-    }
-}
-
-template <class T, int NTW, int MT, int LNV = 0>
-void launch8p(const GemmArgs &g, int nwg, hipStream_t s)
-{
-    constexpr size_t lds = 3 * (64 * MT * 128 + 32 * NTW * 128) + (LNV == 2 ? 64 * MT * 8 : 0);
+            }
+            if (more) {
+                dng::tile_coords(dng::xcd_order(d, ntiles), nbm, nbn, g.pw, mblk, nblk);
+                set_tile();
+                fill_ring();
+            }
+            epilogue(cm, cn, cmblk, cwset);
+            if (!more) return;
+            if constexpr (CS || LNIN) asm volatile("s_waitcnt lgkmcnt(0)" ::: "memory");
+        }
+    }
+}
+
+template <class T, int MODE, int NTW, int MT, bool FUSE, bool CS = false, bool LEAN_ = false, int LNV = 0>
+__global__ __launch_bounds__(512, MT <= 2 ? 2 : 1) void k_gemm8(const GemmArgs g)
+{
+    gemm8_body<T, MODE, NTW, MT, FUSE, CS, LEAN_, LNV, false>(g);
+}
+
+template <class T, int MODE, int NTW, int MT, bool CS = false, bool LEAN_ = false, int LNV = 0>
+__global__ __launch_bounds__(512, 1) void k_gemm8p(const GemmArgs g)
+{
+    gemm8_body<T, MODE, NTW, MT, false, CS, LEAN_, LNV, true>(g);
+}
+
+template <class T, int MODE, int NTW, int MT, bool CS = false, bool LEAN = false, int LNV = 0>
+void launch8p(const GemmArgs &g, hipStream_t s)
+{
+    if constexpr (NTW == 5 && MT == 4) {
+        fprintf(stderr, "gc_dn_gemm: no persistent kernel for 160 x 256 tiles\n");
+        abort();
+    } else {
+    constexpr size_t lds = 3 * (64 * MT * 128 + 32 * NTW * 128) + (LNV == 2 ? 64 * MT * 8 : 0) + (CS ? 32 * NTW * 16 : 0);
     static_assert(lds <= 160 * 1024, "LDS ring");
     static gc::AttrOnce once;
-    gc::ensure_dynamic_lds(once, (const void *)k_gemm8p<T, NTW, MT, LNV>, (int)lds);
-    hipLaunchKernelGGL((k_gemm8p<T, NTW, MT, LNV>), dim3(nwg), dim3(512), lds, s, g);
+    gc::ensure_dynamic_lds(once, (const void *)k_gemm8p<T, MODE, NTW, MT, CS, LEAN, LNV>, (int)lds);
+    hipLaunchKernelGGL((k_gemm8p<T, MODE, NTW, MT, CS, LEAN, LNV>), dim3(g.persist), dim3(512), lds, s, g);
+    }
 }
 
 typedef __attribute__((ext_vector_type(8))) int i32x8;
@@ -2009,6 +1865,14 @@
 void dispatch8ln_m(const GemmArgs &g, int lnv, bool lean, dim3 grid, hipStream_t s)
 {
     if (lnv == 3) { if constexpr (NTW == 5) launch8<T, 3, 5, MT, false, false, false, 3>(g, grid, s); return; }
+    if constexpr (MT >= 2) {
+        if (g.persist > 0) {
+            if (lnv == 1) launch8p<T, 3, NTW, MT, false, true, 1>(g, s);
+            else if (lean) launch8p<T, 3, NTW, MT, false, true, 2>(g, s);
+            else launch8p<T, 3, NTW, MT, false, false, 2>(g, s);
+            return;
+        }
+    }
     if (lnv == 1) launch8<T, 3, NTW, MT, false, false, true, 1>(g, grid, s);
     else if (lean) launch8<T, 3, NTW, MT, false, false, true, 2>(g, grid, s);
     else launch8<T, 3, NTW, MT, false, false, false, 2>(g, grid, s);
@@ -2016,12 +1880,12 @@
 template <class T>
 void dispatch8ln(const GemmArgs &g, int lnv, bool lean, int ntw, int mt, dim3 grid, hipStream_t s)
 {
-    if (lnv == 2 && g.persist > 0 && ntw == 4 && mt == 4) { launch8p<T, 4, 4, 2>(g, g.persist, s); return; }
     if (mt == 1 && ntw == 4) { dispatch8ln_m<T, 4, 1>(g, lnv, lean, grid, s); return; }
     with_wave_tile(ntw, mt, [&](auto ntw_, auto mt_) { dispatch8ln_m<T, decltype(ntw_)::value, decltype(mt_)::value>(g, lnv, lean, grid, s); });
 }
 
-inline bool lean_of(const GemmArgs &g, int mode)
+template <class P>
+inline bool lean_of(const P &g, int mode)
 {
     return !g.geglu && g.act == 0 && !g.out_f32 && !g.out_t && g.out && mode != 1 && (mode != 0 || g.K % 64 == 0) && g.N >= 4 &&
            (!g.rowvec || g.rows_per_batch >= 256);
@@ -2029,6 +1893,7 @@
 template <class T, int NTW, int MT>
 void dispatch8lean_m(const GemmArgs &g, int mode, dim3 grid, hipStream_t s)
 {
+    if (g.persist > 0) { if (mode == 0) launch8p<T, 3, NTW, MT, false, true>(g, s); else launch8p<T, 2, NTW, MT, false, true>(g, s); return; }
     if (mode == 0) launch8<T, 3, NTW, MT, false, false, true>(g, grid, s);
     else if (g.ups) launch8<T, 4, NTW, MT, false, false, true>(g, grid, s);
     else launch8<T, 2, NTW, MT, false, false, true>(g, grid, s);
@@ -2043,6 +1908,7 @@
 template <class T, int NTW, int MT>
 void dispatch8cs_m(const GemmArgs &g, int mode, dim3 grid, hipStream_t s)
 {
+    if (g.persist > 0) { launch8p<T, 2, NTW, MT, true>(g, s); return; }
     if (mode == 0) launch8<T, 3, NTW, MT, false, true>(g, grid, s);
     else if (mode == 1) launch8<T, 1, NTW, MT, false, true>(g, grid, s);
     else launch8<T, 2, NTW, MT, false, true>(g, grid, s);
@@ -2061,6 +1927,7 @@
         else if (mode == 1) launch8<T, 1, NTW, MT, true>(g, grid, s);
         else launch8<T, 2, NTW, MT, true>(g, grid, s);
     } else {
+        if (g.persist > 0) { launch8p<T, 3, NTW, MT>(g, s); return; }
         if (mode == 0) { if (g.K % 64 == 0) launch8<T, 3, NTW, MT, false>(g, grid, s); else launch8<T, 0, NTW, MT, false>(g, grid, s); }
         else if (mode == 1) launch8<T, 1, NTW, MT, false>(g, grid, s);
         else if (g.ups) launch8<T, 4, NTW, MT, false>(g, grid, s); else launch8<T, 2, NTW, MT, false>(g, grid, s);
@@ -2071,7 +1938,6 @@
 {
     if constexpr (!FUSE) {
         if (mt == 1 && ntw == 4 && mode == 0 && g.K % 64 == 0) { launch8<T, 3, 4, 1, false>(g, grid, s); return; }
-        if (g.persist > 0 && ntw == 4 && mt == 4 && mode == 0) { launch8p<T, 4, 4>(g, g.persist, s); return; }
     }
     with_wave_tile(ntw, mt, [&](auto ntw_, auto mt_) { dispatch8m<T, decltype(ntw_)::value, decltype(mt_)::value, FUSE>(g, mode, grid, s); });
 }
```

Result: slower. 10.60 (-2.1%).
